# jaswon/osu-dreamer

Measured on AMD Instinct MI355X. Metric: denoiser train-steps/sec + 50-step sample latents/sec, 1/2/4/8 MI355X, higher is better.
Workload: dtype bf16

## Files before the change

include/osu_dreamer_hip.h:

```cpp
#ifndef OSU_DREAMER_HIP_H
#define OSU_DREAMER_HIP_H

#ifdef __cplusplus
extern "C" {
#endif

enum { OD_F32 = 0, OD_BF16 = 1,
       OD_F32X3 = 2,
       OD_F32X3W = 3,
       OD_F16 = 4 };
enum { OD_EPI_NONE = 0, OD_EPI_SILU = 1 };
enum { OD_ACT_NONE = 0, OD_ACT_SILU = 1 };
enum { OD_ERR_ARG = -1, OD_ERR_ALIGN = -2, OD_ERR_UNSUPPORTED = -3, OD_ERR_COMM = -4 };

int od_version(void);
const char* od_build_source_sha(void);
const char* od_error_string(int code);

int od_gemm_nt(int dtype, const void* A, int lda, const void* W, int ldw, const float* bias, void* C, int ldc,
               int M, int N, int K, int epilogue, int accumulate, void* stream);
int od_gemm_nt_qkrope(int dtype, const void* A, int lda, const void* W, int ldw, const float* bias, void* C, int ldc, int M,
                      int N, int K, const float* wq, const float* wk, const float* table, int L, int H, int hd, float eps,
                      float q_scale, void* stream);
int od_gemm_nt_qkrope_split(int dtype, const void* A, int lda, const void* W, int ldw, const float* bias, void* C, int ldc,
                            void* qk_out, int ldqk, int qk_dtype, int M, int N, int K, const float* wq, const float* wk, const float* table,
                            int L, int H, int hd, float eps, float q_scale, void* stream);
int od_gemm_tn(int dtype, const void* G, int ldg, const void* A, int lda, float* dW, int lddw, float* dbias, int M, int N,
               int K, void* stream);
int od_gemm_tn_blocks(int dtype, const void* G, int ldg, const void* A, int lda, float* dW, int lddw, float* dbias, int M, int N,
                      int K, int n_block, int n_valid, void* stream);
int od_colsum(int dtype, const void* G, int ldg, float* out, int M, int N, void* stream);
int od_pack_weight(int dtype, const float* src, int N, int K, void* dst, int Np, int Kp, int transpose,
                   const int* row_map, void* stream);

int od_linear_small(const float* x, const float* W, const float* b, float* out, float* pre, int B, int N, int K, int act,
                    void* stream);
int od_linear_small_bwd(const float* x, const float* W, const float* pre, const float* dout, float* dpre, float* dW,
                        float* db, float* dx, int accumulate_dx, int B, int N, int K, int act, void* stream);

int od_cl_to_frames(int dtype, const float* src, void* dst, int ldd, int B, int C, int L, void* stream);
int od_proj_in(int dtype, const float* xt, const float* W, const float* bias, void* x, int ldx, int B, int E, int L,
               int D, void* stream);
int od_proj_in_bwd(int dtype, const float* xt, const void* dx, int ldx, float* dW, float* db, int B, int E, int L, int D,
                   void* stream);
int od_silu(int dtype, const void* x, void* y, long n, void* stream);
int od_silu_bwd(int dtype, const void* x, const void* dy, void* dx, long n, void* stream);

int od_rmsnorm_film(int dtype, const void* x, int ldx, const float* ssg, const void* cl, int ldcl, int cl_bcast,
                    void* h, int ldh, float* inv_rms, int B, int L, int C, float eps, void* stream);
int od_rmsnorm_film_bwd(int dtype, const void* x, int ldx, const float* inv_rms, const float* ssg, const void* dh,
                        int lddh, void* dres, int lddres, float* dssg, int B, int L, int C, void* stream);
int od_rmsnorm_gate_residual(int dtype, const void* x, int ldx, const void* h, int ldh, const float* ssg, void* xo,
                             int ldxo, float* inv_rms, int B, int L, int C, float eps, void* stream);
int od_rmsnorm_gate_residual_film(int dtype, const void* x, int ldx, const void* h, int ldh, const float* ssg_a, void* xo, int ldxo,
                                  float* inv_a, const float* ssg_b, const void* cl, int ldcl, int cl_bcast, void* h2, int ldh2,
                                  float* inv_b, int B, int L, int C, float eps, void* stream);
int od_rmsnorm_gate_residual_film_dwconv(int dtype, const void* x, int ldx, const void* h, int ldh, const float* ssg_a, void* xo, int ldxo,
                                         float* inv_a, const float* ssg_b, void* h2, int ldh2, float* inv_b, const float* conv_w,
                                         const float* conv_b, void* y, int ldy, int B, int L, int C, int ksize, float eps, void* stream);
int od_rmsnorm_gate_residual_bwd(int dtype, const void* h, int ldh, const float* inv_rms, const float* ssg,
                                 const void* dy, int lddy, void* dh, int lddh, float* dssg, int B, int L, int C,
                                 void* stream);

int od_rope_table(float* table, int L, int hd, void* stream);
int od_qk_norm_rope(int dtype, const void* qkv, int ldqkv, const float* wq, const float* wk, const float* table,
                    void* qk_out, int ldo, int B, int L, int H, int hd, float eps, float q_scale, void* stream);
int od_qk_norm_rope_bwd(int dtype, const void* qkv, int ldqkv, const float* wq, const float* wk, const float* table,
                        const void* dqk, int lddqk, void* dqkv, int lddqkv, float* dwq, float* dwk, int B, int L,
                        int H, int hd, float eps, float q_scale, void* stream);
int od_flash_attn_fwd(int dtype, const void* q, int ldq, const void* k, int ldk, const void* v, int ldv, void* o, int ldo,
                      float* lse, int B, int H, int L, int hd, float scale, int q_prescaled, void* stream);
int od_flash_attn_fwd_varlen(int dtype, const void* q, int ldq, const void* k, int ldk, const void* v, int ldv, void* o, int ldo,
                             float* lse, const int* lens, int B, int H, int L, int hd, float scale, int q_prescaled, void* stream);
int od_flash_attn_bwd(int dtype, const void* q, int ldq, const void* k, int ldk, const void* v, int ldv, const void* o,
                      int ldo, const void* dout, int lddo, const float* lse, float* delta, void* dq, int lddq, void* dk,
                      int lddk, void* dv, int lddv, int B, int H, int L, int hd, float scale, int q_prescaled, void* stream);
int od_attn_aux_create(void** aux_out);
int od_attn_aux_destroy(void* aux);
int od_flash_attn_bwd_aux(int dtype, const void* q, int ldq, const void* k, int ldk, const void* v, int ldv, const void* o,
                          int ldo, const void* dout, int lddo, const float* lse, float* delta, void* dq, int lddq, void* dk,
                          int lddk, void* dv, int lddv, int B, int H, int L, int hd, float scale, int q_prescaled, void* aux, void* stream);
int od_flash_attn_bwd_fused_ws_bytes(int dtype, int B, int H, int L, long* total_out, long* zero_out);
int od_flash_attn_bwd_fused(int dtype, const void* q, int ldq, const void* k, int ldk, const void* v, int ldv, const void* o, int ldo,
                            const void* dout, int lddo, const float* lse, void* dq, int lddq, void* dk, int lddk, void* dv, int lddv,
                            int B, int H, int L, int hd, float scale, int q_prescaled, void* ws, long ws_bytes, void* stream);
int od_flash_attn_bwd_fused_status(const void* ws, int* err_out, void* stream);
int od_flash_attn_bwd_fused_err_offset(void);
int od_flash_attn_bwd_fused_passes(void);
int od_flash_attn_bwd_fused_prof(void* ws, long* out16);
int od_flash_attn_bwd_passes(void);

int od_dwconv(int dtype, const void* x, int ldx, const float* w, const float* bias, void* y, int ldy, int B, int L,
              int C, int ksize, void* stream);
int od_dwconv_varlen(int dtype, const void* x, int ldx, const float* w, const float* bias, void* y, int ldy, const int* lens,
                     int B, int L, int C, int ksize, void* stream);
int od_dwconv_bwd(int dtype, const void* x, int ldx, const float* w, const void* dy, int lddy, void* dx, int lddx,
                  float* dw, float* db, int B, int L, int C, int ksize, void* stream);
int od_scale_channels(int dtype, void* x, int ldx, const float* scale, int B, int L, int C, void* stream);
int od_swiglu_rmsnorm(int dtype, const void* vg, int ldvg, void* hh, int ldhh, float* inv_rms, int M, int Hf, int Hp,
                      float eps, void* stream);
int od_swiglu_rmsnorm_bwd(int dtype, const void* vg, int ldvg, const float* inv_rms, const void* dhh, int lddhh,
                          void* dvg, int lddvg, int M, int Hf, int Hp, void* stream);

int od_final_norm_proj_out(int dtype, const void* x, int ldx, const float* W, const float* bias, float* v,
                           float* inv_rms, int B, int L, int C, int E, float eps, void* stream);
int od_final_norm_proj_out_bwd(int dtype, const void* x, int ldx, const float* inv_rms, const float* W, const float* dv,
                               void* dx, int lddx, float* dW, float* db, int B, int L, int C, int E, void* stream);
int od_uhead_fwd(const float* xt, const float* w0, const float* b0, const float* w1, const float* b1, const float* w3,
                 const float* b3, const float* w4, const float* b4, float* fsum, int B, int E, int L, int U,
                 void* stream);
int od_uhead_fwd_varlen(const float* xt, const float* w0, const float* b0, const float* w1, const float* b1, const float* w3,
                        const float* b3, const float* w4, const float* b4, float* fsum, const int* lens, int B, int E, int L,
                        int U, void* stream);
int od_uhead_bwd(const float* xt, const float* w0, const float* b0, const float* w1, const float* b1, const float* w3,
                 const float* b3, const float* w4, const float* b4, const float* dfm, float* dw0, float* db0, float* dw1,
                 float* db1, float* dw3, float* db3, float* dw4, float* db4, int B, int E, int L, int U, void* stream);
int od_uhead_tail(const float* fsum, const float* mod, const float* w_out, const float* b_out, float* u, int B, int U,
                  int L, float u_scale, void* stream);
int od_uhead_tail_varlen(const float* fsum, const float* mod, const float* w_out, const float* b_out, float* u, const int* lens,
                         int B, int U, int L, float u_scale, void* stream);
int od_uhead_tail_bwd(const float* fsum, const float* mod, const float* w_out, const float* b_out, const float* du,
                      float* dfm, float* dmod, float* dw_out, float* db_out, int B, int U, int L, float u_scale,
                      void* stream);

int od_make_xt(const float* x0, const float* x1, const float* t, float* xt, float* dsq, int B, int E, int L, void* stream);
int od_loss_grad(const float* xt, const float* x1, const float* u, const float* v, const float* dsq, float* dv,
                 float* sums, int B, int E, int L, float c0, float osl_w, float del_w, void* stream);
int od_loss_finalize(const float* sums, const float* dsq, const float* u, float* out, float* du, int B, float c0,
                     float osl_w, float del_w, void* stream);
int od_sampler_step(float* x, const float* u, const float* v, const float* eta, int B, int E, int L, void* stream);
int od_sampler_eta(const float* u, float* eta, int B, float c0, int num_steps, void* stream);
int od_sampler_eta_groups(const float* u, const int* offs, float* eta, int G, float c0, int num_steps, void* stream);
int od_sampler_step_varlen(float* x, const float* u, const float* v, const float* eta, const int* lens, const int* offs, int G,
                           int B, int E, int L, void* stream);

int od_det_clear(void);
int od_det_register(const float* base, long count, void* shadow_i64);
int od_det_enable(void* table_dev, void* stream);
int od_det_table_bytes(void);
int od_det_flush(float* dst, long count, void* stream);

int od_sqnorm(const float* g, long n, float* out, const int* status, void* stream);
int od_adamw_ema(float* p, const float* g, float* m, float* v, float* ema, long n, float lr, float beta1, float beta2,
                 float eps, float weight_decay, int step, float ema_decay, int ema_mode, const float* gnorm_sq,
                 float max_norm, const int* status, void* stream);

int od_ema_update(float* ema, const float* p, long n, float ema_decay, int ema_mode, void* stream);

int od_style_conditioning(const float* labels, const float* rff_w, const float* rff_b, const float* cond_w,
                          const float* cond_b, const float* null_labels, float* c, int B, int NL, int F, int H,
                          void* stream);
int od_rmsnorm_rows(const float* x, const float* gamma, float* y, int M, int C, float eps, void* stream);

int od_style_conditioning_bwd(const float* labels, const float* rff_w, const float* rff_b, const float* dc, float* dcond_w,
                              float* dcond_b, float* dnull_labels, int B, int NL, int F, int H, void* stream);
int od_rmsnorm_rows_bwd(const float* x, const float* gamma, const float* dy, float* dx, float* dgamma, int M, int C, float eps,
                        int accumulate_dx, void* stream);
int od_cast_rows(int src_dtype, const void* src, int dst_dtype, void* dst, long n, void* stream);

int od_spec_features_conv(int dtype, const float* audio, const float* w1, const float* b1, const float* g1, const float* w2,
                          const float* b2, const float* g2, void* out, int ldo, int B, int F, int L, float eps, void* stream);
int od_rmsnorm_affine_film(int dtype, const void* x, int ldx, const float* gamma, const float* ssg, void* y, int ldy, int B,
                           int L, int C, float eps, int act, void* stream);
int od_rmsnorm_affine_gate_residual(int dtype, const void* x, int ldx, const void* h, int ldh, const float* gamma,
                                    const float* ssg, void* xo, int ldxo, int B, int L, int C, float eps, void* stream);
int od_unet_mixer(int dtype, const void* x, int ldx, const void* p, int ldp, int p_bcast, const void* gx, int ldg,
                  const float* gamma, void* xo, int ldxo, int B, int L, int C, float eps, void* stream);
int od_unet_down(int dtype, const void* x, int ldx, const float* w, const float* bias, void* y, int ldy, int B, int Lo, int C,
                 int stride, void* stream);
int od_unet_up(int dtype, const void* x, int ldx, const float* w, const float* bias, void* y, int ldy, int B, int Li, int C,
               int stride, void* stream);
int od_chart_head(int dtype, const void* x, int ldx, const float* W, const float* bias, float* out, int B, int L, int C, int N,
                  int n_sigmoid, int rms, float eps, void* stream);
int od_attn_pool(int dtype, const void* scores, int lds, const void* values, int ldv, float* out, int B, int L, int Hh, int hd,
                 void* stream);
int od_latent_bwd_block_frames(int C);
int od_rmsnorm_affine_film_bwd(int dtype, const void* x, int ldx, const float* gamma, const float* ssg, const void* dy, int lddy, void* dx,
                               int lddx, int accumulate_dx, float* dgamma, float* dssg, float* ws, long ws_floats, int B, int L, int C,
                               float eps, int act, void* stream);
int od_rmsnorm_affine_gate_residual_bwd(int dtype, const void* h, int ldh, const float* gamma, const float* ssg, const void* dxo, int lddxo,
                                        void* dh, int lddh, float* dgamma, float* dssg, float* ws, long ws_floats, int B, int L, int C,
                                        float eps, void* stream);
int od_unet_mixer_bwd(int dtype, const void* p, int ldp, int p_bcast, const void* gx, int ldg, const float* gamma, const void* dxo,
                      int lddxo, void* dp, int lddp, void* dgx, int lddg, float* dgamma, float* ws, long ws_floats, int B, int L, int C,
                      float eps, void* stream);
int od_unet_down_bwd(int dtype, const void* x, int ldx, const float* w, const void* dy, int lddy, void* dx, int lddx, float* dw, float* db,
                     float* ws, long ws_floats, int B, int Lo, int C, int stride, void* stream);
int od_unet_up_bwd(int dtype, const void* x, int ldx, const float* w, const void* dy, int lddy, void* dx, int lddx, float* dw, float* db,
                   float* ws, long ws_floats, int B, int Li, int C, int stride, void* stream);
int od_chart_head_bwd(int dtype, const void* x, int ldx, const float* W, const float* bias, const float* dout, void* dx, int lddx,
                      float* dW, float* db, float* ws, long ws_floats, int B, int L, int C, int N, int rms, float eps, void* stream);
int od_attn_pool_bwd(int dtype, const void* scores, int lds, const void* values, int ldv, const float* dout, void* dscores, int ldds,
                     void* dvalues, int lddv, int B, int L, int Hh, int hd, void* stream);
int od_spec_features_conv_bwd(int dtype, const float* audio, const float* w1, const float* b1, const float* g1, const float* w2,
                              const float* b2, const float* g2, const void* dout, int ldo, float* dw1, float* db1, float* dg1, float* dw2,
                              float* db2, float* dg2, float* ws, long ws_floats, int B, int F, int L, float eps, void* stream);
int od_add_rows(int dtype, const void* x, void* y, long n, void* stream);
int od_proj_in_bwd_input(int dtype, const void* dx, int ldx, const float* W, float* dxt, int B, int E, int L, int D, void* stream);

int od_mmd_imq(const float* z, const float* prior, float* out, float* dz, float* ws, long ws_floats, int N, int D, void* stream);
int od_scale_by(const float* x, const float* g, float* y, long n, void* stream);
int od_latent_perturb(const float* z, long zsb, long zse, long zsl, const float* s, const float* eps_z, const float* eps_s,
                      const float* u_s, const float* repl, const float* u_span, const float* u_start, float* z_out, float* s_out,
                      void* masked, void* start_span, int B2, int E, int l, int S, float s_noise, float z_noise, float s_mask_frac,
                      float z_mask_frac, int training, void* stream);
int od_latent_perturb_bwd(const float* dz_out, const float* ds_out, const void* masked, const int* start_span, float* dz, float* ds,
                          int B2, int E, int l, int S, void* stream);
int od_latent_loss_block_frames(void);
int od_latent_loss_ws_floats(int B2, int L);
int od_latent_loss(const float* logits, const float* chart, const float* pred_labels, const float* true_labels, const void* masked,
                   const float* s_reg, float* loss_ema, void* ema_init, float* out, float* coef, float* ws, long ws_floats, int B2, int L,
                   float s_reg_weight, int training, void* stream);
int od_latent_loss_bwd(const float* logits, const float* chart, const float* pred_labels, const float* true_labels, const void* masked,
                       const float* coef, const float* g, float* dlogits, float* dlabels, float* ds_reg, int B2, int L,
                       float s_reg_weight, void* stream);

int od_spec_features_conv_varlen(int dtype, const float* audio, const float* w1, const float* b1, const float* g1, const float* w2,
                                 const float* b2, const float* g2, void* out, int ldo, const int* lens, int B, int F, int L, float eps,
                                 void* stream);
int od_rmsnorm_affine_film_varlen(int dtype, const void* x, int ldx, const float* gamma, const float* ssg, void* y, int ldy,
                                  const int* lens, int B, int L, int C, float eps, int act, void* stream);
int od_unet_mixer_varlen(int dtype, const void* x, int ldx, const void* p, int ldp, const int* prow, const void* gx, int ldg,
                         const float* gamma, void* xo, int ldxo, int B, int L, int C, float eps, void* stream);
int od_unet_down_varlen(int dtype, const void* x, int ldx, const float* w, const float* bias, void* y, int ldy, const int* lens,
                        int B, int Lo, int C, int stride, void* stream);
int od_unet_up_varlen(int dtype, const void* x, int ldx, const float* w, const float* bias, void* y, int ldy, const int* lens,
                      int B, int Li, int C, int stride, void* stream);
int od_chart_head_varlen(int dtype, const void* x, int ldx, const float* W, const float* bias, float* out, const int* lens, int B,
                         int L, int C, int N, int n_sigmoid, int rms, float eps, void* stream);
int od_attn_pool_varlen(int dtype, const void* scores, int lds, const void* values, int ldv, float* out, const int* lens, int B,
                        int L, int Hh, int hd, void* stream);

int od_comm_load(const char* path);
int od_comm_version(void);
int od_comm_unique_id(void* out, int nbytes);
int od_comm_init(void** comm_out, int nranks, int rank, const void* unique_id, int nbytes);
int od_comm_destroy(void* comm);
int od_comm_abort(void* comm);
int od_comm_count(void* comm);
int od_comm_ring_standin(float* buf, long count, int channels, int threads, int rounds, void* stream);
int od_allreduce_grads(void* comm, float* grads, long count, int average, void* stream);
int od_broadcast_f32(void* comm, float* buf, long count, int root, void* stream);

int od_graph_begin(void* stream);
int od_graph_end(void* stream, void** graph_exec_out);
int od_graph_launch(void* graph_exec, void* stream);
int od_graph_destroy(void* graph_exec);

int od_mfma_calibrate(float* scratch, int iters, double* flops_out, void* stream);

#ifdef __cplusplus
}
#endif
#endif
```

osu_dreamer_amd/csrc/rowops.hip:

```cpp
#include "od_common.h"
#include "od_api_internal.h"

namespace {

#ifndef OD_QK_BPW
#define OD_QK_BPW 8
#endif
constexpr int ROWS_PER_WAVE_BWD = 16;

template <class T, int NCH>
__device__ __forceinline__ void load_row(const T* row, int C, int lane, float (&v)[NCH][8]) {
#pragma unroll
    for (int i = 0; i < NCH; i++) {
        const int c = (lane + 64 * i) * 8;
        if (c < C) od_ld8(row + c, v[i]);
        else {
#pragma unroll
            for (int e = 0; e < 8; e++) v[i][e] = 0.f;
        }
    }
}
template <int NCH>
__device__ __forceinline__ float row_sumsq(const float (&v)[NCH][8]) {
    float s = 0.f;
#pragma unroll
    for (int i = 0; i < NCH; i++)
#pragma unroll
        for (int e = 0; e < 8; e++) s += v[i][e] * v[i][e];
    return od_wave_sum(s);
}

template <class T, int NCH>
__global__ __launch_bounds__(256) void rmsnorm_film_kernel(const T* __restrict__ x, int ldx, const float* __restrict__ ssg,
                                                           const T* __restrict__ cl, int ldcl, int cl_bcast,
                                                           T* __restrict__ h, int ldh, float* __restrict__ inv_rms,
                                                           int B, int L, int C, float eps) {
    const int lane = threadIdx.x & 63;
    const long m = (long)blockIdx.x * 4 + (threadIdx.x >> 6);
    if (m >= (long)B * L) return;
    const int b = (int)(m / L), l = (int)(m % L);
    float v[NCH][8];
    load_row<T, NCH>(x + m * ldx, C, lane, v);
    const float inv = rsqrtf(row_sumsq<NCH>(v) / (float)C + eps);
    if (lane == 0 && inv_rms) inv_rms[m] = inv;
    const float* sc = ssg + (size_t)b * 3 * C;
    const T* clrow = cl ? cl + (size_t)(cl_bcast ? l : m) * ldcl : nullptr;
#pragma unroll
    for (int i = 0; i < NCH; i++) {
        const int c = (lane + 64 * i) * 8;
        if (c >= C) continue;
        float s[8], sh[8], o[8];
        od_ld8(sc + c, s); od_ld8(sc + C + c, sh);
#pragma unroll
        for (int e = 0; e < 8; e++) o[e] = v[i][e] * inv * (1.f + s[e]) + sh[e];
        if (clrow) {
            float a[8]; od_ld8(clrow + c, a);
#pragma unroll
            for (int e = 0; e < 8; e++) o[e] += a[e];
        }
        od_st8(h + m * ldh + c, o);
    }
}

template <class T, int NCH>
__global__ __launch_bounds__(256) void rmsnorm_film_bwd_kernel(const T* __restrict__ x, int ldx, const float* __restrict__ inv_rms,
                                                               const float* __restrict__ ssg, const T* __restrict__ dh, int lddh,
                                                               T* __restrict__ dres, int lddres, float* __restrict__ dssg,
                                                               int B, int L, int C, const OdDetTable* __restrict__ det) {
    __shared__ float red[2][NCH * 512];
    const int lane = threadIdx.x & 63, wave = threadIdx.x >> 6;
    const int b = blockIdx.y;
    const int l0 = (blockIdx.x * 4 + wave) * ROWS_PER_WAVE_BWD;
    float dsc[NCH][8], dsh[NCH][8], scl[NCH][8];
#pragma unroll
    for (int i = 0; i < NCH; i++) {
        const int c = (lane + 64 * i) * 8;
#pragma unroll
        for (int e = 0; e < 8; e++) { dsc[i][e] = 0.f; dsh[i][e] = 0.f; scl[i][e] = 0.f; }
        if (c < C) od_ld8(ssg + (size_t)b * 3 * C + c, scl[i]);
    }
    for (int r = 0; r < ROWS_PER_WAVE_BWD; r++) {
        const int l = l0 + r;
        if (l >= L) break;
        const long m = (long)b * L + l;
        float xv[NCH][8], gv[NCH][8];
        load_row<T, NCH>(x + m * ldx, C, lane, xv);
        load_row<T, NCH>(dh + m * lddh, C, lane, gv);
        const float inv = inv_rms[m];
        float dot = 0.f;
#pragma unroll
        for (int i = 0; i < NCH; i++)
#pragma unroll
            for (int e = 0; e < 8; e++) {
                const float xh = xv[i][e] * inv;
                dsc[i][e] += gv[i][e] * xh;
                dsh[i][e] += gv[i][e];
                gv[i][e] *= (1.f + scl[i][e]);
                dot += gv[i][e] * xh;
                xv[i][e] = xh;
            }
        dot = od_wave_sum(dot) / (float)C;
#pragma unroll
        for (int i = 0; i < NCH; i++) {
            const int c = (lane + 64 * i) * 8;
            if (c >= C) continue;
            float o[8];
            od_ld8(dres + m * lddres + c, o);
#pragma unroll
            for (int e = 0; e < 8; e++) o[e] += inv * (gv[i][e] - xv[i][e] * dot);
            od_st8(dres + m * lddres + c, o);
        }
    }
    for (int w = 0; w < 4; w++) {
        if (wave == w) {
#pragma unroll
            for (int i = 0; i < NCH; i++)
#pragma unroll
                for (int e = 0; e < 8; e++) {
                    const int idx = (lane + 64 * i) * 8 + e;
                    if (w == 0) { red[0][idx] = dsc[i][e]; red[1][idx] = dsh[i][e]; }
                    else { red[0][idx] += dsc[i][e]; red[1][idx] += dsh[i][e]; }
                }
        }
        __syncthreads();
    }
    for (int c = threadIdx.x; c < C; c += 256) {
        od_red_add(det, dssg + (size_t)b * 3 * C + c, red[0][c]);
        od_red_add(det, dssg + (size_t)b * 3 * C + C + c, red[1][c]);
    }
}

template <class T, int NCH>
__global__ __launch_bounds__(256) void rmsnorm_gate_res_kernel(const T* __restrict__ x, int ldx, const T* __restrict__ h, int ldh,
                                                               const float* __restrict__ ssg, T* __restrict__ xo, int ldxo,
                                                               float* __restrict__ inv_rms, int B, int L, int C, float eps) {
    const int lane = threadIdx.x & 63;
    const long m = (long)blockIdx.x * 4 + (threadIdx.x >> 6);
    if (m >= (long)B * L) return;
    const int b = (int)(m / L);
    float v[NCH][8];
    load_row<T, NCH>(h + m * ldh, C, lane, v);
    const float inv = rsqrtf(row_sumsq<NCH>(v) / (float)C + eps);
    if (lane == 0 && inv_rms) inv_rms[m] = inv;
    const float* gate = ssg + (size_t)b * 3 * C + 2 * C;
#pragma unroll
    for (int i = 0; i < NCH; i++) {
        const int c = (lane + 64 * i) * 8;
        if (c >= C) continue;
        float g[8], o[8];
        od_ld8(gate + c, g);
        od_ld8(x + m * ldx + c, o);
#pragma unroll
        for (int e = 0; e < 8; e++) o[e] += v[i][e] * inv * g[e];
        od_st8(xo + m * ldxo + c, o);
    }
}

template <class T, int NCH>
__global__ __launch_bounds__(256) void rmsnorm_gate_res_film_kernel(const T* __restrict__ x, int ldx, const T* __restrict__ h, int ldh,
                                                                    const float* __restrict__ ssg_a, T* __restrict__ xo, int ldxo,
                                                                    float* __restrict__ inv_a, const float* __restrict__ ssg_b,
                                                                    const T* __restrict__ cl, int ldcl, int cl_bcast,
                                                                    T* __restrict__ h2, int ldh2, float* __restrict__ inv_b,
                                                                    int B, int L, int C, float eps) {
    const int lane = threadIdx.x & 63;
    const long m = (long)blockIdx.x * 4 + (threadIdx.x >> 6);
    if (m >= (long)B * L) return;
    const int b = (int)(m / L), l = (int)(m % L);
    float v[NCH][8];
    load_row<T, NCH>(h + m * ldh, C, lane, v);
    const float inv = rsqrtf(row_sumsq<NCH>(v) / (float)C + eps);
    if (lane == 0 && inv_a) inv_a[m] = inv;
    const float* gate = ssg_a + (size_t)b * 3 * C + 2 * C;
#pragma unroll
    for (int i = 0; i < NCH; i++) {
        const int c = (lane + 64 * i) * 8;
        if (c >= C) {
#pragma unroll
            for (int e = 0; e < 8; e++) v[i][e] = 0.f;
            continue;
        }
        float g[8], o[8];
        od_ld8(gate + c, g);
        od_ld8(x + m * ldx + c, o);
#pragma unroll
        for (int e = 0; e < 8; e++) o[e] += v[i][e] * inv * g[e];
        od_st8(xo + m * ldxo + c, o);
#pragma unroll
        for (int e = 0; e < 8; e++) v[i][e] = od_round_to<T>(o[e]);
    }
    const float inv2 = rsqrtf(row_sumsq<NCH>(v) / (float)C + eps);
    if (lane == 0 && inv_b) inv_b[m] = inv2;
    const float* sc = ssg_b + (size_t)b * 3 * C;
    const T* clrow = cl ? cl + (size_t)(cl_bcast ? l : m) * ldcl : nullptr;
#pragma unroll
    for (int i = 0; i < NCH; i++) {
        const int c = (lane + 64 * i) * 8;
        if (c >= C) continue;
        float s2[8], sh[8], o[8];
        od_ld8(sc + c, s2); od_ld8(sc + C + c, sh);
#pragma unroll
        for (int e = 0; e < 8; e++) o[e] = v[i][e] * inv2 * (1.f + s2[e]) + sh[e];
        if (clrow) {
            float a[8]; od_ld8(clrow + c, a);
#pragma unroll
            for (int e = 0; e < 8; e++) o[e] += a[e];
        }
        od_st8(h2 + m * ldh2 + c, o);
    }
}

template <class T, int KS, int RUN>
__global__ __launch_bounds__(256) void rmsnorm_gate_res_film_dwconv_kernel(const T* __restrict__ x, int ldx, const T* __restrict__ h, int ldh,
                                                                           const float* __restrict__ ssg_a, T* __restrict__ xo, int ldxo,
                                                                           float* __restrict__ inv_a, const float* __restrict__ ssg_b,
                                                                           T* __restrict__ h2, int ldh2, float* __restrict__ inv_b,
                                                                           const float* __restrict__ cw, const float* __restrict__ cb,
                                                                           T* __restrict__ y, int ldy, int B, int L, int C, float eps) {
    constexpr int R = KS / 2;
    const int lane = threadIdx.x & 63;
    const int b = blockIdx.y;
    const int l0 = (blockIdx.x * 4 + (threadIdx.x >> 6)) * RUN;
    if (l0 >= L) return;
    const int c = lane * 8;
    const bool act = c < C;
    float gate[8], sc[8], sh[8], wv[8][KS], bv[8];
#pragma unroll
    for (int e = 0; e < 8; e++) {
        gate[e] = 0.f; sc[e] = 0.f; sh[e] = 0.f; bv[e] = 0.f;
#pragma unroll
        for (int j = 0; j < KS; j++) wv[e][j] = 0.f;
    }
    if (act) {
        od_ld8(ssg_a + (size_t)b * 3 * C + 2 * C + c, gate);
        od_ld8(ssg_b + (size_t)b * 3 * C + c, sc);
        od_ld8(ssg_b + (size_t)b * 3 * C + C + c, sh);
#pragma unroll
        for (int k = 0; k < 8; k++) {
            bv[k] = cb[c + k];
#pragma unroll
            for (int j = 0; j < KS; j++) wv[k][j] = cw[(size_t)(c + k) * KS + j];
        }
    }
    float win[KS][8];
#pragma unroll
    for (int j = 0; j < KS; j++)
#pragma unroll
        for (int e = 0; e < 8; e++) win[j][e] = 0.f;
    const int lend = l0 + RUN < L ? l0 + RUN : L;
    for (int l = l0 - R; l < lend + R; l++) {
#pragma unroll
        for (int e = 0; e < 8; e++) win[KS - 1][e] = 0.f;
        if (l >= 0 && l < L) {
            const long m = (long)b * L + l;
            const bool own = l >= l0 && l < lend;
            float v[1][8], o[8];
            load_row<T, 1>(h + m * ldh, C, lane, v);
            const float inv = rsqrtf(row_sumsq<1>(v) / (float)C + eps);
            if (act) {
                od_ld8(x + m * ldx + c, o);
#pragma unroll
                for (int e = 0; e < 8; e++) o[e] += v[0][e] * inv * gate[e];
                if (own) od_st8(xo + m * ldxo + c, o);
#pragma unroll
                for (int e = 0; e < 8; e++) v[0][e] = od_round_to<T>(o[e]);
            }
            const float inv2 = rsqrtf(row_sumsq<1>(v) / (float)C + eps);
            if (own && lane == 0) {
                if (inv_a) inv_a[m] = inv;
                if (inv_b) inv_b[m] = inv2;
            }
            if (act) {
                float hv[8];
#pragma unroll
                for (int e = 0; e < 8; e++) hv[e] = v[0][e] * inv2 * (1.f + sc[e]) + sh[e];
                if (own && h2) od_st8(h2 + m * ldh2 + c, hv);
#pragma unroll
                for (int e = 0; e < 8; e++) win[KS - 1][e] = od_round_to<T>(hv[e]);
            }
        }
        const int lc = l - R;
        if (lc >= l0 && lc < lend && act) {
            float o[8];
#pragma unroll
            for (int k = 0; k < 8; k++) {
                float s = bv[k];
#pragma unroll
                for (int j = 0; j < KS; j++) s += wv[k][j] * win[j][k];
                o[k] = s;
            }
            od_st8(y + ((size_t)b * L + lc) * ldy + c, o);
        }
#pragma unroll
        for (int j = 0; j < KS - 1; j++)
#pragma unroll
            for (int e = 0; e < 8; e++) win[j][e] = win[j + 1][e];
    }
}

template <class T, int NCH>
__global__ __launch_bounds__(256) void rmsnorm_gate_res_bwd_kernel(const T* __restrict__ h, int ldh, const float* __restrict__ inv_rms,
                                                                   const float* __restrict__ ssg, const T* __restrict__ dy, int lddy,
                                                                   T* __restrict__ dh, int lddh, float* __restrict__ dssg,
                                                                   int B, int L, int C, const OdDetTable* __restrict__ det) {
    __shared__ float red[NCH * 512];
    const int lane = threadIdx.x & 63, wave = threadIdx.x >> 6;
    const int b = blockIdx.y;
    const int l0 = (blockIdx.x * 4 + wave) * ROWS_PER_WAVE_BWD;
    float dg[NCH][8], gate[NCH][8];
#pragma unroll
    for (int i = 0; i < NCH; i++) {
        const int c = (lane + 64 * i) * 8;
#pragma unroll
        for (int e = 0; e < 8; e++) { dg[i][e] = 0.f; gate[i][e] = 0.f; }
        if (c < C) od_ld8(ssg + (size_t)b * 3 * C + 2 * C + c, gate[i]);
    }
    for (int r = 0; r < ROWS_PER_WAVE_BWD; r++) {
        const int l = l0 + r;
        if (l >= L) break;
        const long m = (long)b * L + l;
        float hv[NCH][8], gv[NCH][8];
        load_row<T, NCH>(h + m * ldh, C, lane, hv);
        load_row<T, NCH>(dy + m * lddy, C, lane, gv);
        const float inv = inv_rms[m];
        float dot = 0.f;
#pragma unroll
        for (int i = 0; i < NCH; i++)
#pragma unroll
            for (int e = 0; e < 8; e++) {
                const float hh = hv[i][e] * inv;
                dg[i][e] += gv[i][e] * hh;
                gv[i][e] *= gate[i][e];
                dot += gv[i][e] * hh;
                hv[i][e] = hh;
            }
        dot = od_wave_sum(dot) / (float)C;
#pragma unroll
        for (int i = 0; i < NCH; i++) {
            const int c = (lane + 64 * i) * 8;
            if (c >= C) continue;
            float o[8];
#pragma unroll
            for (int e = 0; e < 8; e++) o[e] = inv * (gv[i][e] - hv[i][e] * dot);
            od_st8(dh + m * lddh + c, o);
        }
    }
    for (int w = 0; w < 4; w++) {
        if (wave == w) {
#pragma unroll
            for (int i = 0; i < NCH; i++)
#pragma unroll
                for (int e = 0; e < 8; e++) {
                    const int idx = (lane + 64 * i) * 8 + e;
                    if (w == 0) red[idx] = dg[i][e]; else red[idx] += dg[i][e];
                }
        }
        __syncthreads();
    }
    for (int c = threadIdx.x; c < C; c += 256) od_red_add(det, dssg + (size_t)b * 3 * C + 2 * C + c, red[c]);
}

template <class T, int NCH>
__global__ __launch_bounds__(256) void swiglu_rmsnorm_kernel(const T* __restrict__ vg, int ldvg, T* __restrict__ hh, int ldhh,
                                                             float* __restrict__ inv_rms, long M, int Hf, int Hp, float eps) {
    const int lane = threadIdx.x & 63;
    const long m = (long)blockIdx.x * 4 + (threadIdx.x >> 6);
    if (m >= M) return;
    float v[NCH][8], g[NCH][8];
    load_row<T, NCH>(vg + m * ldvg, Hp, lane, v);
    load_row<T, NCH>(vg + m * ldvg + Hp, Hp, lane, g);
#pragma unroll
    for (int i = 0; i < NCH; i++)
#pragma unroll
        for (int e = 0; e < 8; e++) v[i][e] *= od_silu(g[i][e]);
    const float inv = rsqrtf(row_sumsq<NCH>(v) / (float)Hf + eps);
    if (lane == 0 && inv_rms) inv_rms[m] = inv;
#pragma unroll
    for (int i = 0; i < NCH; i++) {
        const int c = (lane + 64 * i) * 8;
        if (c >= Hp) continue;
        float o[8];
#pragma unroll
        for (int e = 0; e < 8; e++) o[e] = v[i][e] * inv;
        od_st8(hh + m * ldhh + c, o);
    }
}

template <class T, int NCH>
__global__ __launch_bounds__(256) void swiglu_rmsnorm_bwd_kernel(const T* __restrict__ vg, int ldvg, const float* __restrict__ inv_rms,
                                                                 const T* __restrict__ dhh, int lddhh, T* __restrict__ dvg, int lddvg,
                                                                 long M, int Hf, int Hp) {
    const int lane = threadIdx.x & 63;
    const long m = (long)blockIdx.x * 4 + (threadIdx.x >> 6);
    if (m >= M) return;
    float v[NCH][8], g[NCH][8], d[NCH][8];
    load_row<T, NCH>(vg + m * ldvg, Hp, lane, v);
    load_row<T, NCH>(vg + m * ldvg + Hp, Hp, lane, g);
    load_row<T, NCH>(dhh + m * lddhh, Hp, lane, d);
    const float inv = inv_rms[m];
    float dot = 0.f;
    float sg[NCH][8], gs[NCH][8];
#pragma unroll
    for (int i = 0; i < NCH; i++)
#pragma unroll
        for (int e = 0; e < 8; e++) {
            gs[i][e] = od_sigmoid(g[i][e]);
            sg[i][e] = g[i][e] * gs[i][e];
            dot += d[i][e] * (v[i][e] * sg[i][e] * inv);
        }
    dot = od_wave_sum(dot) / (float)Hf;
#pragma unroll
    for (int i = 0; i < NCH; i++) {
        const int c = (lane + 64 * i) * 8;
        if (c >= Hp) continue;
        float ov[8], og[8];
#pragma unroll
        for (int e = 0; e < 8; e++) {
            const float sh = v[i][e] * sg[i][e] * inv;
            const float ds = inv * (d[i][e] - sh * dot);
            ov[e] = ds * sg[i][e];
            og[e] = ds * v[i][e] * (gs[i][e] * (1.0f + g[i][e] * (1.0f - gs[i][e])));
        }
        od_st8(dvg + m * lddvg + c, ov);
        od_st8(dvg + m * lddvg + Hp + c, og);
    }
}

template <class T, int NCH>
__global__ __launch_bounds__(256) void final_proj_kernel(const T* __restrict__ x, int ldx, const float* __restrict__ W,
                                                         const float* __restrict__ bias, float* __restrict__ vout,
                                                         float* __restrict__ inv_rms, int B, int L, int C, int E, float eps) {
    const int lane = threadIdx.x & 63;
    const long m = (long)blockIdx.x * 4 + (threadIdx.x >> 6);
    if (m >= (long)B * L) return;
    const int b = (int)(m / L), l = (int)(m % L);
    float v[NCH][8];
    load_row<T, NCH>(x + m * ldx, C, lane, v);
    const float inv = rsqrtf(row_sumsq<NCH>(v) / (float)C + eps);
    if (lane == 0 && inv_rms) inv_rms[m] = inv;
    for (int e = 0; e < E; e++) {
        float s = 0.f;
#pragma unroll
        for (int i = 0; i < NCH; i++) {
            const int c = (lane + 64 * i) * 8;
            if (c >= C) continue;
            float w[8]; od_ld8(W + (size_t)e * C + c, w);
#pragma unroll
            for (int k = 0; k < 8; k++) s += w[k] * v[i][k];
        }
        s = od_wave_sum(s) * inv;
        if (lane == 0) vout[((size_t)b * E + e) * L + l] = s + bias[e];
    }
}

template <class T, int NCH>
__global__ __launch_bounds__(256) void final_proj_bwd_kernel(const T* __restrict__ x, int ldx, const float* __restrict__ inv_rms,
                                                             const float* __restrict__ W, const float* __restrict__ dv,
                                                             T* __restrict__ dx, int lddx, float* __restrict__ dW,
                                                             float* __restrict__ db, int B, int L, int C, int E,
                                                             const OdDetTable* __restrict__ det) {
    constexpr int MAXE = 8;
    __shared__ float red[MAXE * NCH * 512];
    __shared__ float redb[4][MAXE];
    const int lane = threadIdx.x & 63, wave = threadIdx.x >> 6;
    const int b = blockIdx.y;
    const int l0 = (blockIdx.x * 4 + wave) * ROWS_PER_WAVE_BWD;
    float wv[MAXE][NCH][8], dw[MAXE][NCH][8], dbv[MAXE];
#pragma unroll
    for (int e = 0; e < MAXE; e++) {
        dbv[e] = 0.f;
#pragma unroll
        for (int i = 0; i < NCH; i++) {
            const int c = (lane + 64 * i) * 8;
#pragma unroll
            for (int k = 0; k < 8; k++) { wv[e][i][k] = 0.f; dw[e][i][k] = 0.f; }
            if (e < E && c < C) od_ld8(W + (size_t)e * C + c, wv[e][i]);
        }
    }
    for (int r = 0; r < ROWS_PER_WAVE_BWD; r++) {
        const int l = l0 + r;
        if (l >= L) break;
        const long m = (long)b * L + l;
        float xv[NCH][8], dn[NCH][8], dve[MAXE];
        load_row<T, NCH>(x + m * ldx, C, lane, xv);
        const float inv = inv_rms[m];
#pragma unroll
        for (int e = 0; e < MAXE; e++) { dve[e] = e < E ? dv[((size_t)b * E + e) * L + l] : 0.f; dbv[e] += dve[e]; }
        float dot = 0.f;
#pragma unroll
        for (int i = 0; i < NCH; i++)
#pragma unroll
            for (int k = 0; k < 8; k++) {
                const float xh = xv[i][k] * inv;
                float s = 0.f;
#pragma unroll
                for (int e = 0; e < MAXE; e++) { s += dve[e] * wv[e][i][k]; dw[e][i][k] += dve[e] * xh; }
                dn[i][k] = s;
                dot += s * xh;
                xv[i][k] = xh;
            }
        dot = od_wave_sum(dot) / (float)C;
#pragma unroll
        for (int i = 0; i < NCH; i++) {
            const int c = (lane + 64 * i) * 8;
            if (c >= C) continue;
            float o[8];
#pragma unroll
            for (int k = 0; k < 8; k++) o[k] = inv * (dn[i][k] - xv[i][k] * dot);
            od_st8(dx + m * lddx + c, o);
        }
    }
    if (lane == 0)
        for (int e = 0; e < MAXE; e++) redb[wave][e] = dbv[e];
    for (int w = 0; w < 4; w++) {
        if (wave == w) {
#pragma unroll
            for (int e = 0; e < MAXE; e++)
#pragma unroll
                for (int i = 0; i < NCH; i++)
#pragma unroll
                    for (int k = 0; k < 8; k++) {
                        const int idx = e * NCH * 512 + (lane + 64 * i) * 8 + k;
                        if (w == 0) red[idx] = dw[e][i][k]; else red[idx] += dw[e][i][k];
                    }
        }
        __syncthreads();
    }
    for (int e = 0; e < E; e++)
        for (int c = threadIdx.x; c < C; c += 256) od_red_add(det, dW + (size_t)e * C + c, red[e * NCH * 512 + c]);
    if (threadIdx.x < E) od_red_add(det, db + threadIdx.x, redb[0][threadIdx.x] + redb[1][threadIdx.x] + redb[2][threadIdx.x] + redb[3][threadIdx.x]);
}

template <class T, class TO = T>
__global__ __launch_bounds__(256) void qk_norm_rope_kernel(const T* __restrict__ qkv, int ldqkv, const float* __restrict__ wq,
                                                           const float* __restrict__ wk, const float* __restrict__ table,
                                                           TO* __restrict__ out, int ldo, int B, int L, int H, int hd, float eps,
                                                           float q_scale) {
    const int lane = threadIdx.x & 63;
    const long m = (long)blockIdx.x * 4 + (threadIdx.x >> 6);
    if (m >= (long)B * L) return;
    const int l = (int)(m % L);
    const int lph = hd / 8, half = lph / 2;
    const int nchunks = 2 * H * lph;
    const int niter = (nchunks + 63) / 64;
    for (int it = 0; it < niter; it++) {
        const int q = it * 64 + lane;
        const bool act = q < nchunks;
        const int slot = q / lph, c8 = q % lph;
        float v[8];
        if (act) od_ld8(qkv + m * ldqkv + (size_t)slot * hd + c8 * 8, v);
        else {
#pragma unroll
            for (int e = 0; e < 8; e++) v[e] = 0.f;
        }
        float ss = 0.f;
#pragma unroll
        for (int e = 0; e < 8; e++) ss += v[e] * v[e];
        for (int msk = 1; msk < lph; msk <<= 1) ss += __shfl_xor(ss, msk);
        const float inv = rsqrtf(ss / (float)hd + eps);
        const float* w = (slot < H ? wq : wk) + c8 * 8;
        float y[8], p[8];
#pragma unroll
        for (int e = 0; e < 8; e++) y[e] = act ? v[e] * inv * w[e] : 0.f;
#pragma unroll
        for (int e = 0; e < 8; e++) p[e] = __shfl_xor(y[e], half);
        if (act) {
            const bool first = c8 < half;
            const int j0 = (c8 % half) * 8;
            const float* tb = table + ((size_t)l * (hd / 2) + j0) * 2;
            float o[8];
#pragma unroll
            for (int e = 0; e < 8; e++) {
                const float cs = tb[2 * e], sn = tb[2 * e + 1];
                o[e] = (first ? (y[e] * cs - p[e] * sn) : (p[e] * sn + y[e] * cs)) * (slot < H ? q_scale : 1.f);
            }
            od_st8(out + m * ldo + (size_t)slot * hd + c8 * 8, o);
        }
    }
}

template <class T>
__global__ __launch_bounds__(256) void qk_norm_rope_bwd_kernel(const T* __restrict__ qkv, int ldqkv, const float* __restrict__ wq,
                                                               const float* __restrict__ wk, const float* __restrict__ table,
                                                               const T* __restrict__ dqk, int lddqk, T* __restrict__ dqkv, int lddqkv,
                                                               float* __restrict__ dwq, float* __restrict__ dwk,
                                                               int B, int L, int H, int hd, float eps, float q_scale,
                                                               const OdDetTable* __restrict__ det) {
    __shared__ long long sdw[2][256];
    __shared__ int s_bad;
    const int lane = threadIdx.x & 63, wave = threadIdx.x >> 6;
    for (int i = threadIdx.x; i < 512; i += 256) sdw[i >> 8][i & 255] = 0;
    if (threadIdx.x == 0) s_bad = 0;
    __syncthreads();
    const int lph = hd / 8, half = lph / 2;
    const int nchunks = 2 * H * lph;
    const int niter = (nchunks + 63) / 64;
    float aq[8], ak[8];
#pragma unroll
    for (int e = 0; e < 8; e++) { aq[e] = 0.f; ak[e] = 0.f; }
    const long M = (long)B * L;
    const long mbase = ((long)blockIdx.x * 4 + wave) * ROWS_PER_WAVE_BWD;
    for (int r = 0; r < ROWS_PER_WAVE_BWD; r++) {
        const long m = mbase + r;
        if (m >= M) break;
        const int l = (int)(m % L);
        for (int it = 0; it < niter; it++) {
            const int q = it * 64 + lane;
            const bool act = q < nchunks;
            const int slot = q / lph, c8 = q % lph;
            float v[8], d[8];
            if (act) {
                od_ld8(qkv + m * ldqkv + (size_t)slot * hd + c8 * 8, v); od_ld8(dqk + m * lddqk + (size_t)slot * hd + c8 * 8, d);
                if (slot < H) {
#pragma unroll
                    for (int e = 0; e < 8; e++) d[e] *= q_scale;
                }
            } else {
#pragma unroll
                for (int e = 0; e < 8; e++) { v[e] = 0.f; d[e] = 0.f; }
            }
            float ss = 0.f;
#pragma unroll
            for (int e = 0; e < 8; e++) ss += v[e] * v[e];
            for (int msk = 1; msk < lph; msk <<= 1) ss += __shfl_xor(ss, msk);
            const float inv = rsqrtf(ss / (float)hd + eps);
            float p[8], dy[8];
#pragma unroll
            for (int e = 0; e < 8; e++) p[e] = __shfl_xor(d[e], half);
            const bool first = c8 < half;
            const int j0 = (c8 % (half > 0 ? half : 1)) * 8;
            const float* tb = table + ((size_t)l * (hd / 2) + j0) * 2;
            const float* w = (slot < H ? wq : wk) + c8 * 8;
            float dot = 0.f;
#pragma unroll
            for (int e = 0; e < 8; e++) {
                const float cs = act ? tb[2 * e] : 0.f, sn = act ? tb[2 * e + 1] : 0.f;
                dy[e] = first ? (d[e] * cs + p[e] * sn) : (-p[e] * sn + d[e] * cs);
                const float xh = v[e] * inv;
                const float wv = act ? w[e] : 0.f;
                if (act) { if (slot < H) aq[e] += dy[e] * xh; else ak[e] += dy[e] * xh; }
                dy[e] *= wv;
                dot += dy[e] * xh;
                v[e] = xh;
            }
            for (int msk = 1; msk < lph; msk <<= 1) dot += __shfl_xor(dot, msk);
            dot /= (float)hd;
            if (act) {
                float o[8];
#pragma unroll
                for (int e = 0; e < 8; e++) o[e] = inv * (dy[e] - v[e] * dot);
                od_st8(dqkv + m * lddqkv + (size_t)slot * hd + c8 * 8, o);
            }
        }
    }
    const int c8 = lane % lph;
#pragma unroll
    for (int e = 0; e < 8; e++) {
        od_lds_fix_add(&sdw[0][c8 * 8 + e], aq[e], &s_bad);
        od_lds_fix_add(&sdw[1][c8 * 8 + e], ak[e], &s_bad);
    }
    __syncthreads();
    if (threadIdx.x < hd) {
        od_red_add(det, dwq + threadIdx.x, od_lds_unfix(sdw[0][threadIdx.x], s_bad));
        od_red_add(det, dwk + threadIdx.x, od_lds_unfix(sdw[1][threadIdx.x], s_bad));
    }
}

template <class T, int LPH, int NIT>
__global__ __launch_bounds__(256) void qk_norm_rope_pos_kernel(const T* __restrict__ qkv, int ldqkv, const float* __restrict__ wq,
                                                               const float* __restrict__ wk, const float* __restrict__ table,
                                                               T* __restrict__ out, int ldo, int B, int L, float eps, float q_scale,
                                                               int bpw, int lpw) {
    constexpr int HD = 8 * LPH, HALFL = LPH / 2;
    const int lane = threadIdx.x & 63, c8 = lane % LPH;
    const int wpl = (B + bpw - 1) / bpw;
    const long gw = (long)blockIdx.x * 4 + (threadIdx.x >> 6);
    const int l0 = (int)(gw / wpl) * lpw, b0 = (int)(gw % wpl) * bpw;
    if (l0 >= L) return;
    const int l1 = l0 + lpw < L ? l0 + lpw : L, b1 = b0 + bpw < B ? b0 + bpw : B;
    float w[2][8];
    od_ld8(wq + c8 * 8, w[0]); od_ld8(wk + c8 * 8, w[1]);
#pragma unroll
    for (int e = 0; e < 8; e++) w[0][e] *= q_scale;
    const bool first = c8 < HALFL;
    for (int l = l0; l < l1; l++) {
        float tb[16];
        const float* tp = table + ((size_t)l * (HD / 2) + (c8 % HALFL) * 8) * 2;
        od_ld8(tp, *(float(*)[8])&tb[0]); od_ld8(tp + 8, *(float(*)[8])&tb[8]);
        float cs[8], sn[8];
#pragma unroll
        for (int e = 0; e < 8; e++) { cs[e] = tb[2 * e]; sn[e] = first ? -tb[2 * e + 1] : tb[2 * e + 1]; }
        for (int b = b0; b < b1; b++) {
            const long m = (long)b * L + l;
            float v[NIT][8];
#pragma unroll
            for (int it = 0; it < NIT; it++) od_ld8(qkv + m * ldqkv + (size_t)(it * 64 + lane) * 8, v[it]);
#pragma unroll
            for (int it = 0; it < NIT; it++) {
                float ss = 0.f;
#pragma unroll
                for (int e = 0; e < 8; e++) ss += v[it][e] * v[it][e];
#pragma unroll
                for (int msk = 1; msk < LPH; msk <<= 1) ss += __shfl_xor(ss, msk);
                const float inv = rsqrtf(ss / (float)HD + eps);
                const float* wv = w[it < NIT / 2 ? 0 : 1];
                float y[8], o[8];
#pragma unroll
                for (int e = 0; e < 8; e++) y[e] = v[it][e] * inv * wv[e];
#pragma unroll
                for (int e = 0; e < 8; e++) o[e] = y[e] * cs[e] + __shfl_xor(y[e], HALFL) * sn[e];
                od_st8(out + m * ldo + (size_t)(it * 64 + lane) * 8, o);
            }
        }
    }
}

template <class T, int LPH, int NIT>
__global__ __launch_bounds__(256) void qk_norm_rope_pos_bwd_kernel(const T* __restrict__ qkv, int ldqkv, const float* __restrict__ wq,
                                                                   const float* __restrict__ wk, const float* __restrict__ table,
                                                                   const T* __restrict__ dqk, int lddqk, T* __restrict__ dqkv, int lddqkv,
                                                                   float* __restrict__ dwq, float* __restrict__ dwk,
                                                                   int B, int L, float eps, float q_scale, int bpw, int lpw,
                                                                   const OdDetTable* __restrict__ det) {
    constexpr int HD = 8 * LPH, HALFL = LPH / 2;
    __shared__ long long s_dw[2][HD];
    __shared__ int s_bad;
    for (int i = threadIdx.x; i < 2 * HD; i += 256) s_dw[i / HD][i % HD] = 0;
    if (threadIdx.x == 0) s_bad = 0;
    __syncthreads();
    const int lane = threadIdx.x & 63, c8 = lane % LPH;
    const int wpl = (B + bpw - 1) / bpw;
    const long gw = (long)blockIdx.x * 4 + (threadIdx.x >> 6);
    const int l0 = (int)(gw / wpl) * lpw, b0 = (int)(gw % wpl) * bpw;
    const int l1 = l0 + lpw < L ? l0 + lpw : L, b1 = b0 + bpw < B ? b0 + bpw : B;
    float w[2][8], acc[2][8];
    od_ld8(wq + c8 * 8, w[0]); od_ld8(wk + c8 * 8, w[1]);
#pragma unroll
    for (int e = 0; e < 8; e++) { acc[0][e] = 0.f; acc[1][e] = 0.f; }
    const bool first = c8 < HALFL;
    for (int l = l0; l < l1; l++) {
        float tb[16];
        const float* tp = table + ((size_t)l * (HD / 2) + (c8 % HALFL) * 8) * 2;
        od_ld8(tp, *(float(*)[8])&tb[0]); od_ld8(tp + 8, *(float(*)[8])&tb[8]);
        float cs[8], sn[8];
#pragma unroll
        for (int e = 0; e < 8; e++) { cs[e] = tb[2 * e]; sn[e] = first ? tb[2 * e + 1] : -tb[2 * e + 1]; }
        for (int b = b0; b < b1; b++) {
            const long m = (long)b * L + l;
            float v[NIT][8], d[NIT][8];
#pragma unroll
            for (int it = 0; it < NIT; it++) {
                od_ld8(qkv + m * ldqkv + (size_t)(it * 64 + lane) * 8, v[it]);
                od_ld8(dqk + m * lddqk + (size_t)(it * 64 + lane) * 8, d[it]);
            }
#pragma unroll
            for (int it = 0; it < NIT; it++) {
                const int qk = it < NIT / 2 ? 0 : 1;
                const float gs = qk == 0 ? q_scale : 1.f;
                float ss = 0.f;
#pragma unroll
                for (int e = 0; e < 8; e++) ss += v[it][e] * v[it][e];
#pragma unroll
                for (int msk = 1; msk < LPH; msk <<= 1) ss += __shfl_xor(ss, msk);
                const float inv = rsqrtf(ss / (float)HD + eps);
                float dy[8], xh[8], dot = 0.f;
#pragma unroll
                for (int e = 0; e < 8; e++) d[it][e] *= gs;
#pragma unroll
                for (int e = 0; e < 8; e++) {
                    const float u = d[it][e] * cs[e] + __shfl_xor(d[it][e], HALFL) * sn[e];
                    xh[e] = v[it][e] * inv;
                    acc[qk][e] += u * xh[e];
                    dy[e] = u * w[qk][e];
                    dot += dy[e] * xh[e];
                }
#pragma unroll
                for (int msk = 1; msk < LPH; msk <<= 1) dot += __shfl_xor(dot, msk);
                dot /= (float)HD;
                float o[8];
#pragma unroll
                for (int e = 0; e < 8; e++) o[e] = inv * (dy[e] - xh[e] * dot);
                od_st8(dqkv + m * lddqkv + (size_t)(it * 64 + lane) * 8, o);
            }
        }
    }
#pragma unroll
    for (int msk = LPH; msk < 64; msk <<= 1)
#pragma unroll
        for (int e = 0; e < 8; e++) { acc[0][e] += __shfl_xor(acc[0][e], msk); acc[1][e] += __shfl_xor(acc[1][e], msk); }
    if (lane < LPH) {
#pragma unroll
        for (int e = 0; e < 8; e++) { od_lds_fix_add(&s_dw[0][c8 * 8 + e], acc[0][e], &s_bad); od_lds_fix_add(&s_dw[1][c8 * 8 + e], acc[1][e], &s_bad); }
    }
    __syncthreads();
    if (threadIdx.x < HD) {
        od_red_add(det, dwq + threadIdx.x, od_lds_unfix(s_dw[0][threadIdx.x], s_bad));
        od_red_add(det, dwk + threadIdx.x, od_lds_unfix(s_dw[1][threadIdx.x], s_bad));
    }
}

__global__ void rope_table_kernel(float* __restrict__ table, int L, int hd) {
    const long i = (long)blockIdx.x * blockDim.x + threadIdx.x;
    const int half = hd / 2;
    if (i >= (long)L * half) return;
    const int l = (int)(i / half), j = (int)(i % half);
    const float e = (float)(2 * j) / (float)(-hd);
    const float inv_freq = (float)pow(10000.0, (double)e);
    const float ang = (float)l * inv_freq;
    table[2 * i] = cosf(ang);
    table[2 * i + 1] = sinf(ang);
}

inline int nch_for(int C) { return (C + 511) / 512; }

inline void qk_pos_split(int B, int L, int& bpw, int& lpw) {
    bpw = B < OD_QK_BPW ? B : OD_QK_BPW;
    lpw = OD_QK_BPW / bpw;
    if (lpw < 1) lpw = 1;
    (void)L;
}

}

#define DISPATCH_T_NCH(DT, NCHV, CALL)                                          \
    do {                                                                        \
        if ((DT) == OD_BF16) {                                                  \
            typedef bf16_t T_;                                                  \
            if ((NCHV) == 1) { constexpr int N_ = 1; CALL; }                    \
            else if ((NCHV) == 2) { constexpr int N_ = 2; CALL; }               \
            else if ((NCHV) == 3) { constexpr int N_ = 3; CALL; }               \
            else return OD_ERR_UNSUPPORTED;                                     \
        } else if ((DT) == OD_F32) {                                            \
            typedef float T_;                                                   \
            if ((NCHV) == 1) { constexpr int N_ = 1; CALL; }                    \
            else if ((NCHV) == 2) { constexpr int N_ = 2; CALL; }               \
            else if ((NCHV) == 3) { constexpr int N_ = 3; CALL; }               \
            else return OD_ERR_UNSUPPORTED;                                     \
        } else return OD_ERR_ARG;                                               \
    } while (0)

extern "C" int od_rmsnorm_film(int dtype, const void* x, int ldx, const float* ssg, const void* cl, int ldcl, int cl_bcast,
                               void* h, int ldh, float* inv_rms, int B, int L, int C, float eps, void* stream) {
    if (C % 8 || ldx % 8 || ldh % 8 || (cl && ldcl % 8)) return OD_ERR_ALIGN;
    const long M = (long)B * L;
    dim3 grid((unsigned)((M + 3) / 4));
    DISPATCH_T_NCH(dtype, nch_for(C),
        OD_LAUNCH((rmsnorm_film_kernel<T_, N_>), grid, dim3(256), 0, (hipStream_t)stream, (const T_*)x, ldx, ssg, (const T_*)cl, ldcl,
                  cl_bcast, (T_*)h, ldh, inv_rms, B, L, C, eps));
    OD_CHECK_LAUNCH();
    return 0;
}

extern "C" int od_rmsnorm_film_bwd(int dtype, const void* x, int ldx, const float* inv_rms, const float* ssg, const void* dh,
                                   int lddh, void* dres, int lddres, float* dssg, int B, int L, int C, void* stream) {
    if (C % 8 || ldx % 8 || lddh % 8 || lddres % 8) return OD_ERR_ALIGN;
    dim3 grid((L + 4 * ROWS_PER_WAVE_BWD - 1) / (4 * ROWS_PER_WAVE_BWD), B);
    DISPATCH_T_NCH(dtype, nch_for(C),
        OD_LAUNCH((rmsnorm_film_bwd_kernel<T_, N_>), grid, dim3(256), 0, (hipStream_t)stream, (const T_*)x, ldx, inv_rms, ssg,
                  (const T_*)dh, lddh, (T_*)dres, lddres, dssg, B, L, C, od_det_active()));
    OD_CHECK_LAUNCH();
    return 0;
}

extern "C" int od_rmsnorm_gate_residual(int dtype, const void* x, int ldx, const void* h, int ldh, const float* ssg, void* xo,
                                        int ldxo, float* inv_rms, int B, int L, int C, float eps, void* stream) {
    if (C % 8 || ldx % 8 || ldh % 8 || ldxo % 8) return OD_ERR_ALIGN;
    const long M = (long)B * L;
    dim3 grid((unsigned)((M + 3) / 4));
    DISPATCH_T_NCH(dtype, nch_for(C),
        OD_LAUNCH((rmsnorm_gate_res_kernel<T_, N_>), grid, dim3(256), 0, (hipStream_t)stream, (const T_*)x, ldx, (const T_*)h, ldh, ssg,
                  (T_*)xo, ldxo, inv_rms, B, L, C, eps));
    OD_CHECK_LAUNCH();
    return 0;
}

extern "C" int od_rmsnorm_gate_residual_film(int dtype, const void* x, int ldx, const void* h, int ldh, const float* ssg_a, void* xo,
                                             int ldxo, float* inv_a, const float* ssg_b, const void* cl, int ldcl, int cl_bcast,
                                             void* h2, int ldh2, float* inv_b, int B, int L, int C, float eps, void* stream) {
    if (C % 8 || ldx % 8 || ldh % 8 || ldxo % 8 || ldh2 % 8 || (cl && ldcl % 8)) return OD_ERR_ALIGN;
    const long M = (long)B * L;
    dim3 grid((unsigned)((M + 3) / 4));
    DISPATCH_T_NCH(dtype, nch_for(C),
        OD_LAUNCH((rmsnorm_gate_res_film_kernel<T_, N_>), grid, dim3(256), 0, (hipStream_t)stream, (const T_*)x, ldx, (const T_*)h, ldh,
                  ssg_a, (T_*)xo, ldxo, inv_a, ssg_b, (const T_*)cl, ldcl, cl_bcast, (T_*)h2, ldh2, inv_b, B, L, C, eps));
    OD_CHECK_LAUNCH();
    return 0;
}

extern "C" int od_rmsnorm_gate_residual_film_dwconv(int dtype, const void* x, int ldx, const void* h, int ldh, const float* ssg_a, void* xo,
                                                    int ldxo, float* inv_a, const float* ssg_b, void* h2, int ldh2, float* inv_b,
                                                    const float* conv_w, const float* conv_b, void* y, int ldy, int B, int L, int C,
                                                    int ksize, float eps, void* stream) {
    if (C % 8 || ldx % 8 || ldh % 8 || ldxo % 8 || (h2 && ldh2 % 8) || ldy % 8) return OD_ERR_ALIGN;
    if (C > 512 || (ksize != 3 && ksize != 5 && ksize != 7 && ksize != 9)) return OD_ERR_UNSUPPORTED;
    if (!x || !h || !xo || !y || !conv_w || !conv_b || xo == x || xo == h) return OD_ERR_ARG;
#ifndef OD_FD_SMALL_RUNS
#define OD_FD_SMALL_RUNS 2048
#endif
    const bool small = (long)B * ((L + 31) / 32) < OD_FD_SMALL_RUNS;
    const int run = small ? 8 : 32;
    dim3 grid((unsigned)((L + 4 * run - 1) / (4 * run)), (unsigned)B);
#define FD_GO2(T_, KS_, RUN_) OD_LAUNCH((rmsnorm_gate_res_film_dwconv_kernel<T_, KS_, RUN_>), grid, dim3(256), 0, (hipStream_t)stream, (const T_*)x, ldx, \
                   (const T_*)h, ldh, ssg_a, (T_*)xo, ldxo, inv_a, ssg_b, (T_*)h2, ldh2, inv_b, conv_w, conv_b, (T_*)y, ldy, B, L, C, eps)
#define FD_GO1(T_, KS_) do { if (small) FD_GO2(T_, KS_, 8); else FD_GO2(T_, KS_, 32); } while (0)
#define FD_GO(KS_) do { if (dtype == OD_BF16) FD_GO1(bf16_t, KS_); else if (dtype == OD_F32) FD_GO1(float, KS_); else return OD_ERR_UNSUPPORTED; } while (0)
    if (ksize == 5) FD_GO(5); else if (ksize == 3) FD_GO(3); else if (ksize == 7) FD_GO(7); else FD_GO(9);
#undef FD_GO
#undef FD_GO1
#undef FD_GO2
    OD_CHECK_LAUNCH();
    return 0;
}

extern "C" int od_rmsnorm_gate_residual_bwd(int dtype, const void* h, int ldh, const float* inv_rms, const float* ssg,
                                            const void* dy, int lddy, void* dh, int lddh, float* dssg, int B, int L, int C,
                                            void* stream) {
    if (C % 8 || ldh % 8 || lddy % 8 || lddh % 8) return OD_ERR_ALIGN;
    dim3 grid((L + 4 * ROWS_PER_WAVE_BWD - 1) / (4 * ROWS_PER_WAVE_BWD), B);
    DISPATCH_T_NCH(dtype, nch_for(C),
        OD_LAUNCH((rmsnorm_gate_res_bwd_kernel<T_, N_>), grid, dim3(256), 0, (hipStream_t)stream, (const T_*)h, ldh, inv_rms, ssg,
                  (const T_*)dy, lddy, (T_*)dh, lddh, dssg, B, L, C, od_det_active()));
    OD_CHECK_LAUNCH();
    return 0;
}

extern "C" int od_swiglu_rmsnorm(int dtype, const void* vg, int ldvg, void* hh, int ldhh, float* inv_rms, int M, int Hf, int Hp,
                                 float eps, void* stream) {
    if (Hp % 8 || ldvg % 8 || ldhh % 8 || Hf > Hp) return OD_ERR_ALIGN;
    dim3 grid((unsigned)((M + 3) / 4));
    DISPATCH_T_NCH(dtype, nch_for(Hp),
        OD_LAUNCH((swiglu_rmsnorm_kernel<T_, N_>), grid, dim3(256), 0, (hipStream_t)stream, (const T_*)vg, ldvg, (T_*)hh, ldhh, inv_rms,
                  (long)M, Hf, Hp, eps));
    OD_CHECK_LAUNCH();
    return 0;
}

extern "C" int od_swiglu_rmsnorm_bwd(int dtype, const void* vg, int ldvg, const float* inv_rms, const void* dhh, int lddhh,
                                     void* dvg, int lddvg, int M, int Hf, int Hp, void* stream) {
    if (Hp % 8 || ldvg % 8 || lddhh % 8 || lddvg % 8 || Hf > Hp) return OD_ERR_ALIGN;
    dim3 grid((unsigned)((M + 3) / 4));
    DISPATCH_T_NCH(dtype, nch_for(Hp),
        OD_LAUNCH((swiglu_rmsnorm_bwd_kernel<T_, N_>), grid, dim3(256), 0, (hipStream_t)stream, (const T_*)vg, ldvg, inv_rms,
                  (const T_*)dhh, lddhh, (T_*)dvg, lddvg, (long)M, Hf, Hp));
    OD_CHECK_LAUNCH();
    return 0;
}

extern "C" int od_final_norm_proj_out(int dtype, const void* x, int ldx, const float* W, const float* bias, float* v,
                                      float* inv_rms, int B, int L, int C, int E, float eps, void* stream) {
    if (C % 8 || ldx % 8) return OD_ERR_ALIGN;
    if (E > 8 || C > 1024) return OD_ERR_UNSUPPORTED;
    const long M = (long)B * L;
    dim3 grid((unsigned)((M + 3) / 4));
    DISPATCH_T_NCH(dtype, nch_for(C),
        OD_LAUNCH((final_proj_kernel<T_, N_>), grid, dim3(256), 0, (hipStream_t)stream, (const T_*)x, ldx, W, bias, v, inv_rms, B, L, C, E, eps));
    OD_CHECK_LAUNCH();
    return 0;
}

extern "C" int od_final_norm_proj_out_bwd(int dtype, const void* x, int ldx, const float* inv_rms, const float* W,
                                          const float* dv, void* dx, int lddx, float* dW, float* db, int B, int L, int C, int E,
                                          void* stream) {
    if (C % 8 || ldx % 8 || lddx % 8) return OD_ERR_ALIGN;
    if (E > 8 || C > 512) return OD_ERR_UNSUPPORTED;
    dim3 grid((L + 4 * ROWS_PER_WAVE_BWD - 1) / (4 * ROWS_PER_WAVE_BWD), B);
    if (dtype == OD_BF16)
        OD_LAUNCH((final_proj_bwd_kernel<bf16_t, 1>), grid, dim3(256), 0, (hipStream_t)stream, (const bf16_t*)x, ldx, inv_rms, W, dv,
                  (bf16_t*)dx, lddx, dW, db, B, L, C, E, od_det_active());
    else
        OD_LAUNCH((final_proj_bwd_kernel<float, 1>), grid, dim3(256), 0, (hipStream_t)stream, (const float*)x, ldx, inv_rms, W, dv,
                  (float*)dx, lddx, dW, db, B, L, C, E, od_det_active());
    OD_CHECK_LAUNCH();
    return 0;
}

extern "C" int od_rope_table(float* table, int L, int hd, void* stream) {
    if (hd % 2 || L <= 0) return OD_ERR_ARG;
    const long n = (long)L * (hd / 2);
    OD_LAUNCH(rope_table_kernel, dim3((unsigned)((n + 255) / 256)), dim3(256), 0, (hipStream_t)stream, table, L, hd);
    OD_CHECK_LAUNCH();
    return 0;
}

extern "C" int od_qk_norm_rope(int dtype, const void* qkv, int ldqkv, const float* wq, const float* wk, const float* table,
                               void* qk_out, int ldo, int B, int L, int H, int hd, float eps, float q_scale, void* stream) {
    if (hd % 16 || hd > 256 || 64 % (hd / 8)) return OD_ERR_UNSUPPORTED;
    if (ldqkv % 8 || ldo % 8) return OD_ERR_ALIGN;
    const long M = (long)B * L;
    const int lph = hd / 8;
    if (dtype != OD_F16 && (lph == 4 || lph == 8) && (H * lph) % 64 == 0 && ldqkv >= 2 * H * hd) {
        const int nit = 2 * H * lph / 64;
        if (nit == 2 || nit == 4 || nit == 8) {
            int bpw, lpw; qk_pos_split(B, L, bpw, lpw);
            const long waves = (long)((L + lpw - 1) / lpw) * ((B + bpw - 1) / bpw);
            dim3 g2((unsigned)((waves + 3) / 4));
#define QKP(TT, LPHV, NITV) OD_LAUNCH((qk_norm_rope_pos_kernel<TT, LPHV, NITV>), g2, dim3(256), 0, (hipStream_t)stream, (const TT*)qkv, ldqkv, wq, wk, table, (TT*)qk_out, ldo, B, L, eps, q_scale, bpw, lpw)
#define QKP_T(TT) do { if (lph == 8) { if (nit == 2) QKP(TT, 8, 2); else if (nit == 4) QKP(TT, 8, 4); else QKP(TT, 8, 8); } \
                       else { if (nit == 2) QKP(TT, 4, 2); else if (nit == 4) QKP(TT, 4, 4); else QKP(TT, 4, 8); } } while (0)
            if (dtype == OD_BF16) QKP_T(bf16_t); else QKP_T(float);
#undef QKP_T
#undef QKP
            OD_CHECK_LAUNCH();
            return 0;
        }
    }
    dim3 grid((unsigned)((M + 3) / 4));
    if (dtype == OD_F16)
        OD_LAUNCH((qk_norm_rope_kernel<bf16_t, f16_t>), grid, dim3(256), 0, (hipStream_t)stream, (const bf16_t*)qkv, ldqkv, wq, wk, table,
                  (f16_t*)qk_out, ldo, B, L, H, hd, eps, q_scale);
    else if (dtype == OD_BF16)
        OD_LAUNCH((qk_norm_rope_kernel<bf16_t>), grid, dim3(256), 0, (hipStream_t)stream, (const bf16_t*)qkv, ldqkv, wq, wk, table,
                  (bf16_t*)qk_out, ldo, B, L, H, hd, eps, q_scale);
    else
        OD_LAUNCH((qk_norm_rope_kernel<float>), grid, dim3(256), 0, (hipStream_t)stream, (const float*)qkv, ldqkv, wq, wk, table,
                  (float*)qk_out, ldo, B, L, H, hd, eps, q_scale);
    OD_CHECK_LAUNCH();
    return 0;
}

extern "C" int od_qk_norm_rope_bwd(int dtype, const void* qkv, int ldqkv, const float* wq, const float* wk, const float* table,
                                   const void* dqk, int lddqk, void* dqkv, int lddqkv, float* dwq, float* dwk, int B, int L,
                                   int H, int hd, float eps, float q_scale, void* stream) {
    if (hd % 16 || hd > 256 || 64 % (hd / 8)) return OD_ERR_UNSUPPORTED;
    if (ldqkv % 8 || lddqk % 8 || lddqkv % 8) return OD_ERR_ALIGN;
    const long M = (long)B * L;
    const int lph = hd / 8;
    if ((lph == 4 || lph == 8) && (H * lph) % 64 == 0) {
        const int nit = 2 * H * lph / 64;
        if (nit == 2 || nit == 4 || nit == 8) {
            int bpw, lpw; qk_pos_split(B, L, bpw, lpw);
            lpw *= 4;
            const long waves = (long)((L + lpw - 1) / lpw) * ((B + bpw - 1) / bpw);
            dim3 g2((unsigned)((waves + 3) / 4));
#define QKPB(TT, LPHV, NITV) OD_LAUNCH((qk_norm_rope_pos_bwd_kernel<TT, LPHV, NITV>), g2, dim3(256), 0, (hipStream_t)stream, (const TT*)qkv, ldqkv, wq, wk, table, (const TT*)dqk, lddqk, (TT*)dqkv, lddqkv, dwq, dwk, B, L, eps, q_scale, bpw, lpw, od_det_active())
#define QKPB_T(TT) do { if (lph == 8) { if (nit == 2) QKPB(TT, 8, 2); else if (nit == 4) QKPB(TT, 8, 4); else QKPB(TT, 8, 8); } \
                        else { if (nit == 2) QKPB(TT, 4, 2); else if (nit == 4) QKPB(TT, 4, 4); else QKPB(TT, 4, 8); } } while (0)
            if (dtype == OD_BF16) QKPB_T(bf16_t); else QKPB_T(float);
#undef QKPB_T
#undef QKPB
            OD_CHECK_LAUNCH();
            return 0;
        }
    }
    dim3 grid((unsigned)((M + 4 * ROWS_PER_WAVE_BWD - 1) / (4 * ROWS_PER_WAVE_BWD)));
    if (dtype == OD_BF16)
        OD_LAUNCH((qk_norm_rope_bwd_kernel<bf16_t>), grid, dim3(256), 0, (hipStream_t)stream, (const bf16_t*)qkv, ldqkv, wq, wk, table,
                  (const bf16_t*)dqk, lddqk, (bf16_t*)dqkv, lddqkv, dwq, dwk, B, L, H, hd, eps, q_scale, od_det_active());
    else
        OD_LAUNCH((qk_norm_rope_bwd_kernel<float>), grid, dim3(256), 0, (hipStream_t)stream, (const float*)qkv, ldqkv, wq, wk, table,
                  (const float*)dqk, lddqk, (float*)dqkv, lddqkv, dwq, dwk, B, L, H, hd, eps, q_scale, od_det_active());
    OD_CHECK_LAUNCH();
    return 0;
}
```

osu_dreamer_amd/engine.py:

```python
from __future__ import annotations


import math
import os
from typing import Dict, List, Optional

import torch

from . import det, ops
from ._lib import OD_ACT_NONE, OD_ACT_SILU

OD_FUSE_FILM_DWCONV_DEFAULT = "0"

FP32_EPS = float(torch.finfo(torch.float32).eps)


def _ceil(x: int, m: int) -> int:
    return (x + m - 1) // m * m


class Workspace:

    def __init__(self, device):
        self.device = device
        self.t: Dict[str, torch.Tensor] = {}
        self.bytes = 0

    def get(self, name: str, shape, dtype) -> torch.Tensor:
        t = self.t.get(name)
        if t is None:
            t = torch.zeros(shape, dtype=dtype, device=self.device)
            self.t[name] = t
            self.bytes += t.numel() * t.element_size()
            if name in det.WS_NAMES:
                ctx = det.context(self.device)
                if ctx is not None:
                    ctx.register(t)
        return t


class DenoiserEngine:
    def __init__(self, model):
        self.model = model
        a = model.args
        ba = a.backbone_args
        self.E, self.A, self.S = model.emb_dim, model.a_dim, model.style_dim
        self.Cg, self.D, self.U = a.global_cond_dim, a.backbone_dim, a.u_head_dim
        self.H, self.hd, self.depth = ba.n_heads, ba.head_dim, ba.depth
        self.dh = self.H * self.hd
        self.q_scale = math.log2(math.e) / math.sqrt(self.hd)
        self.radius = ba.radius
        self.ksize = 1 + 2 * ba.radius
        self.Hf = int(self.D * ba.expand * 2 / 3)
        self.Hp = _ceil(self.Hf, 64)
        if ba.radius not in (0, 1, 2, 3, 4):
            raise NotImplementedError("depthwise kernel sizes 3, 5, 7, 9 (radius 1-4) are compiled; radius 0 is the identity")
        if not (0.0 <= ba.dropout < 1.0):
            raise ValueError(f"dropout probability has to be in [0, 1), got {ba.dropout}")
        self.dropout = float(ba.dropout)
        self._packed: Dict[str, torch.Tensor] = {}
        self._packed_key = None
        self._plan_key = None
        self.ws: Optional[Workspace] = None
        self._rowmap = None
        self.generation = 0
        self._attn_aux = None
        self._attn_ws_cache: Dict[tuple, "ops.FusedAttnBwdWorkspace"] = {}
        self._attn_ws = None
        self.varlen = False
        self.attn_f16 = False

    def _det_flush(self, *tensors):
        ctx = det.context(self.model.arena.data.device)
        if ctx is not None:
            for t in tensors:
                ctx.flush(t)

    def _det_flush_segment(self, name: str):
        ctx = det.context(self.model.arena.data.device)
        if ctx is not None:
            s, e = self.model.arena.segments(self.depth)[name]
            ctx.flush(self.model.arena.ensure_grad()[s:e])

    def P(self, name: str) -> torch.Tensor:
        return self.model.arena.view(name)

    def G(self, name: str) -> torch.Tensor:
        return self.model.arena.grad_view(name)

    def _gemm_weights(self) -> List[str]:
        names = ["proj_audio.0"]
        for i in range(self.depth):
            p = f"net.layers.{i}."
            names += [p + "proj_cl", p + "attn.qkv_proj", p + "attn.out_proj", p + "ffn.proj_vg.1", p + "ffn.proj_o"]
        return names

    def pack_weights(self, dtype: torch.dtype, train: bool, x3: bool = False):
        dev = self.model.arena.data.device
        x3 = bool(x3 and dtype == torch.float32 and not train)
        key = (dtype, train, dev, x3)
        if self._packed_key != key:
            self._packed = {}
            self._packed_key = key
            self.generation += 1
            Hf, Hp = self.Hf, self.Hp
            rm = [-1] * (2 * Hp)
            for j in range(Hf):
                rm[j] = j
                rm[Hp + j] = Hf + j
            self._rowmap = torch.tensor(rm, dtype=torch.int32, device=dev)
        pk = self._packed
        for n in self._gemm_weights():
            w = self.P(n + ".weight")
            N, K = w.shape[0], w.shape[1]
            Np, Kp, rmap = N, K, None
            if n.endswith("ffn.proj_vg.1"):
                Np, rmap = 2 * self.Hp, self._rowmap
            if n.endswith("ffn.proj_o"):
                Kp = self.Hp
            if n not in pk:
                pk[n] = torch.empty(Np, Kp, dtype=dtype, device=dev)
                if x3 and Kp % 32 == 0:
                    pk[n] = ops.SplitWeight(pk[n])
                if train:
                    pk[n + ".T"] = torch.empty(Kp, Np, dtype=dtype, device=dev)
                if rmap is not None:
                    pk[n + ".b"] = torch.empty(Np, dtype=torch.float32, device=dev)
            ops.pack_weight(w, pk[n], row_map=rmap)
            if train:
                ops.pack_weight(w, pk[n + ".T"], transpose=True, row_map=rmap)
            if rmap is not None:
                ops.pack_weight(self.P(n + ".bias"), pk[n + ".b"].view(Np, 1), row_map=rmap)

    def W(self, name: str, T: bool = False) -> torch.Tensor:
        return self._packed[name + (".T" if T else "")]

    def plain_gemm(self, A: torch.Tensor, W: torch.Tensor, bias, C: torch.Tensor):
        ops.gemm_nt(A, W, bias, C, x3=self.x3)

    def plan(self, B: int, L: int, Ba: int, dtype: torch.dtype, train: bool, x3: bool = False, lens=None, offs=None):
        dev = self.model.arena.data.device
        assert not (x3 and train), "the f32x3 product exists for the forward kernels only"
        varlen = lens is not None
        assert not (varlen and train), "the varlen forward exists for no-grad paths only"
        x3 = bool(x3 and dtype == torch.float32)
        ngroups = len(offs) - 1 if offs is not None else 0
        key = (B, L, Ba, dtype, train, dev, x3, getattr(self.model, "attn_dtype", None), varlen, ngroups)
        if key != self._plan_key:
            self.ws = Workspace(dev)
            self._plan_key = key
            self.generation += 1
            tab = self.ws.get("rope", (L, self.hd // 2, 2), torch.float32)
            ops.rope_table(tab, L, self.hd)
        self.varlen = varlen
        if varlen:
            lens_t = torch.as_tensor(lens).to("cpu", torch.int32)
            if lens_t.shape != (B,) or int(lens_t.min()) < 1 or int(lens_t.max()) > L:
                raise ValueError(f"lens must hold B = {B} lengths in [1, {L}]")
            self.ws.get("vl.lens", (B,), torch.int32).copy_(lens_t)
            if offs is not None:
                offs_t = torch.as_tensor(offs).to("cpu", torch.int32)
                if int(offs_t[0]) != 0 or int(offs_t[-1]) != B or bool((offs_t[1:] <= offs_t[:-1]).any()):
                    raise ValueError("offs must rise strictly from 0 to B")
                self.ws.get("vl.offs", (ngroups + 1,), torch.int32).copy_(offs_t)
        self.B, self.L, self.Ba, self.dtype, self.train, self.x3 = B, L, Ba, dtype, train, x3
        self.M, self.Ma = B * L, Ba * L
        self.attn_f16 = getattr(self.model, "attn_dtype", None) == torch.float16
        if self.attn_f16 and (dtype != torch.bfloat16 or self.hd != 64):
            if not getattr(self, "_warned_f16_fallback", False):
                import warnings
                warnings.warn(f"attn_dtype = float16 applies to compute_dtype bfloat16 with head_dim 64; this plan (dtype {dtype}, head_dim "
                              f"{self.hd}) runs its attention in {dtype}")
                self._warned_f16_fallback = True
            self.attn_f16 = False
        return self.ws

    def buf(self, name, shape, dtype=None):
        return self.ws.get(name, shape, self.dtype if dtype is None else dtype)

    def lbuf(self, name, i, shape, dtype=None):
        return self.buf(f"{name}.{i}" if self.train else name, shape, dtype)

    def conditioning(self, audio: torch.Tensor, style: torch.Tensor):
        B, Ba, L = self.B, self.Ba, self.L
        D, A, Cg, U = self.D, self.A, self.Cg, self.U
        f32 = torch.float32
        a_t = self.buf("a_t", (self.Ma, A))
        a_pre = self.buf("a_pre", (self.Ma, A))
        a = self.buf("a", (self.Ma, A))
        ops.cl_to_frames(audio, a_t)
        ops.gemm_nt(a_t, self.W("proj_audio.0"), self.P("proj_audio.0.bias"), a_pre, x3=self.x3)
        ops.silu(a_pre, a)
        cg, cg_pre = self.buf("cg", (B, Cg), f32), self.buf("cg_pre", (B, Cg), f32)
        ops.linear_small(style, self.P("proj_style.0.weight"), self.P("proj_style.0.bias"), cg, cg_pre, OD_ACT_SILU)
        for i in range(self.depth):
            p = f"net.layers.{i}."
            for s in ("ssg1", "ssg2"):
                ops.linear_small(cg, self.P(p + s + ".weight"), self.P(p + s + ".bias"),
                                 self.buf(f"{s}.{i}", (B, 3 * D), f32))
            if not self.train:
                ops.gemm_nt(a, self.W(p + "proj_cl"), self.P(p + "proj_cl.bias"), self.buf(f"cl.{i}", (self.Ma, D)), x3=self.x3)
        ops.linear_small(cg, self.P("u_mod.weight"), self.P("u_mod.bias"), self.buf("umod", (B, 2 * U), f32))

    def pred(self, xt: torch.Tensor, u: torch.Tensor, v: torch.Tensor):
        B, L, M, D, dh, Hp = self.B, self.L, self.M, self.D, self.dh, self.Hp
        f32 = torch.float32
        tab = self.ws.t["rope"]
        bcast = self.Ba == 1 and B > 1
        x = self.lbuf("x_in", 0, (M, D))
        ops.proj_in(xt, self.P("proj_in.weight"), self.P("proj_in.bias"), x)

        def cl_of(i):
            if not self.train:
                return self.ws.t[f"cl.{i}"]
            cl = self.buf("cl", (self.Ma, D))
            ops.gemm_nt(self.ws.t["a"], self.W(f"net.layers.{i}.proj_cl"), self.P(f"net.layers.{i}.proj_cl.bias"), cl)
            return cl

        h1 = self.lbuf("h1", 0, (M, D))
        ops.rmsnorm_film(x, self.ws.t["ssg1.0"], cl_of(0), bcast, h1, self.lbuf("inv1", 0, (M,), f32), B, L)
        for i in range(self.depth):
            p = f"net.layers.{i}."
            ssg1, ssg2 = self.ws.t[f"ssg1.{i}"], self.ws.t[f"ssg2.{i}"]
            qkv = self.lbuf("qkv", i, (M, 3 * dh))
            if self.train or self.attn_f16 or self.hd not in (32, 64) or (2 * dh) % 128:
                qk = self.lbuf("qk16" if self.attn_f16 else "qk", i, (M, 2 * dh), torch.float16 if self.attn_f16 else None)
                ops.gemm_nt_qkrope_split(h1, self.W(p + "attn.qkv_proj"), self.P(p + "attn.qkv_proj.bias"), qkv, qk,
                                         self.P(p + "attn.q_norm.weight"), self.P(p + "attn.k_norm.weight"), tab, L, self.H,
                                         self.hd, FP32_EPS, x3=self.x3, q_scale=self.q_scale)
            else:
                ops.gemm_nt_qkrope(h1, self.W(p + "attn.qkv_proj"), self.P(p + "attn.qkv_proj.bias"), qkv,
                                   self.P(p + "attn.q_norm.weight"), self.P(p + "attn.k_norm.weight"), tab, L,
                                   self.H, self.hd, FP32_EPS, x3=self.x3, q_scale=self.q_scale)
                qk = qkv
            y = self.lbuf("y", i, (M, dh))
            lse = self.lbuf("lse", i, (B, self.H, L), f32)
            if self.varlen:
                ops.flash_attn_fwd_varlen(qk[:, :dh], qk[:, dh:], self._v_of(qkv), y, lse, self.ws.t["vl.lens"], B, self.H, L, self.hd,
                                          1.0 / math.sqrt(self.hd), x3=self.x3, q_prescaled=True)
            else:
                ops.flash_attn_fwd(qk[:, :dh], qk[:, dh:], self._v_of(qkv), y, lse, B, self.H, L, self.hd,
                                   1.0 / math.sqrt(self.hd), x3=self.x3, q_prescaled=True)
            ao = self.lbuf("ao", i, (M, D))
            self.plain_gemm(y, self.W(p + "attn.out_proj"), self.P(p + "attn.out_proj.bias"), ao)
            x_mid = self.lbuf("x_mid", i, (M, D))
            h2 = self.lbuf("h2", i, (M, D))
            fuse_dw = (self.radius > 0 and not self.varlen and D <= 512 and x.data_ptr() != x_mid.data_ptr() and x.dtype in (torch.bfloat16, torch.float32)
                       and os.environ.get("OD_FUSE_FILM_DWCONV", OD_FUSE_FILM_DWCONV_DEFAULT) == "1")
            if fuse_dw:
                hdw = self.lbuf("hdw", i, (M, D))
                ops.rmsnorm_gate_residual_film_dwconv(x, ao, ssg1, x_mid, self.lbuf("inv2", i, (M,), f32), ssg2, h2 if self.train else None,
                                                      self.lbuf("inv3", i, (M,), f32),
                                                      self.P(p + "ffn.proj_vg.0.weight"), self.P(p + "ffn.proj_vg.0.bias"), hdw, B, L, self.ksize)
            else:
                ops.rmsnorm_gate_residual_film(x, ao, ssg1, x_mid, self.lbuf("inv2", i, (M,), f32), ssg2, None, False, h2,
                                               self.lbuf("inv3", i, (M,), f32), B, L)
            if fuse_dw:
                pass
            elif self.radius > 0:
                hdw = self.lbuf("hdw", i, (M, D))
                if self.varlen:
                    ops.dwconv_varlen(h2, self.P(p + "ffn.proj_vg.0.weight"), self.P(p + "ffn.proj_vg.0.bias"), hdw, self.ws.t["vl.lens"], B, L,
                                      self.ksize)
                else:
                    ops.dwconv(h2, self.P(p + "ffn.proj_vg.0.weight"), self.P(p + "ffn.proj_vg.0.bias"), hdw, B, L, self.ksize)
            else:
                hdw = h2
            vg = self.lbuf("vg", i, (M, 2 * Hp))
            ops.gemm_nt(hdw, self.W(p + "ffn.proj_vg.1"), self._packed[p + "ffn.proj_vg.1.b"], vg, x3=self.x3)
            hh = self.lbuf("hh", i, (M, Hp))
            ops.swiglu_rmsnorm(vg, hh, self.lbuf("inv4", i, (M,), f32), self.Hf, Hp)
            if self._drop_active():
                ops.scale_channels(hh, self.draw_dropout_mask(i), B, L)
            fo = self.lbuf("fo", i, (M, D))
            self.plain_gemm(hh, self.W(p + "ffn.proj_o"), self.P(p + "ffn.proj_o.bias"), fo)
            x = self.buf(f"x_in.{i + 1}", (M, D)) if self.train else self.buf(f"x_in.{(i + 1) & 1}", (M, D))
            if i + 1 < self.depth:
                h1 = self.lbuf("h1", i + 1, (M, D))
                ops.rmsnorm_gate_residual_film(x_mid, fo, ssg2, x, self.lbuf("inv5", i, (M,), f32),
                                               self.ws.t[f"ssg1.{i + 1}"], cl_of(i + 1), bcast, h1,
                                               self.lbuf("inv1", i + 1, (M,), f32), B, L)
            else:
                ops.rmsnorm_gate_residual(x_mid, fo, ssg2, x, self.lbuf("inv5", i, (M,), f32), B, L)
        self._x_last = x
        ops.final_norm_proj_out(x, self.P("proj_out.weight"), self.P("proj_out.bias"), v,
                                self.buf("invf", (M,), f32), B, L)
        fsum = self.buf("fsum", (B, self.U), f32)
        fsum.zero_()
        if self.varlen:
            ops.uhead_fwd_varlen(xt, self._uhead_w(), fsum, self.ws.t["vl.lens"], self.U)
            self._det_flush(fsum)
            ops.uhead_tail_varlen(fsum, self.ws.t["umod"], self.P("u_out.weight"), self.P("u_out.bias"), u, self.ws.t["vl.lens"], L,
                                  self.model.u_scale)
        else:
            ops.uhead_fwd(xt, self._uhead_w(), fsum, self.U)
            self._det_flush(fsum)
            ops.uhead_tail(fsum, self.ws.t["umod"], self.P("u_out.weight"), self.P("u_out.bias"), u, L, self.model.u_scale)

    def _v_of(self, qkv: torch.Tensor) -> torch.Tensor:
        v = qkv[:, 2 * self.dh:]
        return v.view(torch.float16) if self.attn_f16 else v

    def attn_bwd_passes(self) -> int:
        from . import _lib
        return int(_lib.lib().cdll.od_flash_attn_bwd_fused_passes() if self.fused_attn_bwd() else _lib.lib().cdll.od_flash_attn_bwd_passes())

    def fused_attn_bwd(self) -> bool:
        import os
        if self.dtype != torch.bfloat16 or self.hd != 64:
            return False
        if self.attn_f16:
            return True
        env = os.environ.get("OD_ATTN_BWD_FUSED", "")
        if env in ("0", "1"):
            return env == "1"
        return self.L >= 2048

    def attn_bwd_launch(self, i: int, dy: torch.Tensor, delta: torch.Tensor, dqkv: torch.Tensor, core_only: bool = False):
        t, dh, p = self.ws.t, self.dh, f"net.layers.{i}."
        qk, qkv, y, lse = t[f"qk16.{i}" if self.attn_f16 else f"qk.{i}"], t[f"qkv.{i}"], t[f"y.{i}"], t[f"lse.{i}"]
        wq, wk = self.P(p + "attn.q_norm.weight"), self.P(p + "attn.k_norm.weight")
        gq, gk = self.G(p + "attn.q_norm.weight"), self.G(p + "attn.k_norm.weight")
        scale = 1.0 / math.sqrt(self.hd)
        dqk = self.buf("d.qk", (self.M, 2 * dh))
        if self.fused_attn_bwd():
            key = (self.B, self.H, self.L, qk.device, qk.dtype)
            ws = self._attn_ws_cache.get(key)
            if ws is None:
                if len(self._attn_ws_cache) >= 4:
                    self._attn_ws_cache.pop(next(iter(self._attn_ws_cache)))
                ws = self._attn_ws_cache[key] = ops.FusedAttnBwdWorkspace(self.B, self.H, self.L, qk.device, qk.dtype)
                ws.checked = False
            self._attn_ws = ws
            ops.flash_attn_bwd_fused(qk[:, :dh], qk[:, dh:], self._v_of(qkv), y, dy, lse, dqk[:, :dh], dqk[:, dh:], dqkv[:, 2 * dh:],
                                     self.B, self.H, self.L, self.hd, scale, self._attn_ws, q_prescaled=True)
        else:
            if (self._attn_aux is None or self._attn_aux.device != qk.device) and qk.is_cuda:
                if self._attn_aux is not None:
                    self._attn_aux.close()
                with torch.cuda.device(qk.device):
                    self._attn_aux = ops.AttnAux()
                self._attn_aux.device = qk.device
            ops.flash_attn_bwd(qk[:, :dh], qk[:, dh:], qkv[:, 2 * dh:], y, dy, lse, delta, dqk[:, :dh], dqk[:, dh:],
                               dqkv[:, 2 * dh:], self.B, self.H, self.L, self.hd, scale, q_prescaled=True, aux=self._attn_aux)
        if not core_only:
            ops.qk_norm_rope_bwd(qkv, wq, wk, t["rope"], dqk, dqkv, gq, gk, self.B, self.L, self.H, self.hd, FP32_EPS, q_scale=self.q_scale)

    def _drop_active(self) -> bool:
        return self.dropout > 0.0 and self.model.training

    def _drop_mask(self, i: int) -> torch.Tensor:
        return self.ws.t[f"drop.{i}"]

    def draw_dropout_mask(self, i: int) -> torch.Tensor:
        keep = 1.0 - self.dropout
        m = self.buf(f"drop.{i}", (self.B, self.Hp), torch.float32)
        m.zero_()
        m[:, :self.Hf] = torch.empty(self.B, self.Hf, device=m.device, dtype=torch.float32).bernoulli_(keep) / keep
        return m

    def _uhead_w(self, grads=False):
        f = self.G if grads else self.P
        return [f(f"u_head.{j}.{s}") for j in (0, 1, 3, 4) for s in ("weight", "bias")]

    def backward(self, xt: torch.Tensor, style: torch.Tensor, du: torch.Tensor, dv: torch.Tensor, reducer=None):
        assert self.train
        B, L, M, D, dh, Hf, Hp, A = self.B, self.L, self.M, self.D, self.dh, self.Hf, self.Hp, self.A
        f32 = torch.float32
        dctx = det.context(self.model.arena.data.device)
        if dctx is not None:
            dctx.register(self.model.arena.ensure_grad())
        tab = self.ws.t["rope"]
        cg, a = self.ws.t["cg"], self.ws.t["a"]
        dx = self.buf("d.x", (M, D))
        dbr = self.buf("d.branch", (M, D))
        dtmp = self.buf("d.tmp", (M, D))
        dhh = self.buf("d.hh", (M, Hp))
        dvg = self.buf("d.vg", (M, 2 * Hp))
        dy = self.buf("d.y", (M, dh))
        dqkv = self.buf("d.qkv", (M, 3 * dh))
        da = self.buf("d.a", (self.Ma, A))
        delta = self.buf("d.delta", (B, self.H, L), f32)
        dcg = self.buf("d.cg", (B, self.Cg), f32)
        dssg1, dssg2 = self.buf("d.ssg1", (B, 3 * D), f32), self.buf("d.ssg2", (B, 3 * D), f32)

        ops.final_norm_proj_out_bwd(self._x_last, self.ws.t["invf"], self.P("proj_out.weight"), dv, dx,
                                    self.G("proj_out.weight"), self.G("proj_out.bias"), B, L)
        dfm, dmod = self.buf("d.fm", (B, self.U), f32), self.buf("d.mod", (B, 2 * self.U), f32)
        ops.uhead_tail_bwd(self.ws.t["fsum"], self.ws.t["umod"], self.P("u_out.weight"), self.P("u_out.bias"), du,
                           dfm, dmod, self.G("u_out.weight"), self.G("u_out.bias"), L, self.model.u_scale)
        ops.uhead_bwd(xt, self._uhead_w(), dfm, self._uhead_w(grads=True), self.U)
        ops.linear_small_bwd(cg, self.P("u_mod.weight"), None, dmod, self.buf("d.lin_pre_umod", (B, 2 * self.U), f32),
                             self.G("u_mod.weight"), self.G("u_mod.bias"), dcg, False, OD_ACT_NONE)
        self._det_flush_segment("tail")
        if reducer is not None:
            reducer.segment_done("tail")

        for i in reversed(range(self.depth)):
            p = f"net.layers.{i}."
            t = self.ws.t
            ssg1, ssg2 = t[f"ssg1.{i}"], t[f"ssg2.{i}"]
            dssg1.zero_()
            dssg2.zero_()
            ops.rmsnorm_gate_residual_bwd(t[f"fo.{i}"], t[f"inv5.{i}"], ssg2, dx, dbr, dssg2, B, L)
            ops.gemm_tn(dbr, t[f"hh.{i}"], self.G(p + "ffn.proj_o.weight"), n_cols=D, k_cols=Hf,
                        dbias=self.G(p + "ffn.proj_o.bias"))
            ops.gemm_nt(dbr, self.W(p + "ffn.proj_o", T=True), None, dhh)
            if self._drop_active():
                ops.scale_channels(dhh, self._drop_mask(i), B, L)
            ops.swiglu_rmsnorm_bwd(t[f"vg.{i}"], t[f"inv4.{i}"], dhh, dvg, Hf, Hp)
            gw, gb = self.G(p + "ffn.proj_vg.1.weight"), self.G(p + "ffn.proj_vg.1.bias")
            hdw = t[f"hdw.{i}"] if self.radius > 0 else t[f"h2.{i}"]
            ops.gemm_tn(dvg, hdw, gw, n_cols=2 * Hp, k_cols=D, dbias=gb, n_block=Hp, n_valid=Hf)
            if self.radius > 0:
                self.plain_gemm(dvg, self.W(p + "ffn.proj_vg.1", T=True), None, dtmp)
                ops.dwconv_bwd(t[f"h2.{i}"], self.P(p + "ffn.proj_vg.0.weight"), dtmp, dbr,
                               self.G(p + "ffn.proj_vg.0.weight"), self.G(p + "ffn.proj_vg.0.bias"), B, L, self.ksize)
            else:
                self.plain_gemm(dvg, self.W(p + "ffn.proj_vg.1", T=True), None, dbr)
            ops.rmsnorm_film_bwd(t[f"x_mid.{i}"], t[f"inv3.{i}"], ssg2, dbr, dx, dssg2, B, L)
            ops.rmsnorm_gate_residual_bwd(t[f"ao.{i}"], t[f"inv2.{i}"], ssg1, dx, dbr, dssg1, B, L)
            ops.gemm_tn(dbr, t[f"y.{i}"], self.G(p + "attn.out_proj.weight"), dbias=self.G(p + "attn.out_proj.bias"))
            ops.gemm_nt(dbr, self.W(p + "attn.out_proj", T=True), None, dy)
            self.attn_bwd_launch(i, dy, delta, dqkv)
            ops.gemm_tn(dqkv, t[f"h1.{i}"], self.G(p + "attn.qkv_proj.weight"), dbias=self.G(p + "attn.qkv_proj.bias"))
            self.plain_gemm(dqkv, self.W(p + "attn.qkv_proj", T=True), None, dtmp)
            ops.gemm_tn(dtmp, a, self.G(p + "proj_cl.weight"), dbias=self.G(p + "proj_cl.bias"))
            ops.gemm_nt(dtmp, self.W(p + "proj_cl", T=True), None, da, accumulate=(i != self.depth - 1))
            ops.rmsnorm_film_bwd(t[f"x_in.{i}"], t[f"inv1.{i}"], ssg1, dtmp, dx, dssg1, B, L)
            lp = self.buf("d.lin_pre_ssg", (B, 3 * D), f32)
            self._det_flush(dssg1, dssg2)
            ops.linear_small_bwd(cg, self.P(p + "ssg2.weight"), None, dssg2, lp, self.G(p + "ssg2.weight"),
                                 self.G(p + "ssg2.bias"), dcg, True, OD_ACT_NONE)
            ops.linear_small_bwd(cg, self.P(p + "ssg1.weight"), None, dssg1, lp, self.G(p + "ssg1.weight"),
                                 self.G(p + "ssg1.bias"), dcg, True, OD_ACT_NONE)
            self._det_flush_segment(f"layer{i}")
            if reducer is not None:
                reducer.segment_done(f"layer{i}")

        ops.proj_in_bwd(xt, dx, self.G("proj_in.weight"), self.G("proj_in.bias"))
        da_pre = self.buf("d.a_pre", (self.Ma, A))
        ops.silu_bwd(self.ws.t["a_pre"], da, da_pre)
        ops.gemm_tn(da_pre, self.ws.t["a_t"], self.G("proj_audio.0.weight"), dbias=self.G("proj_audio.0.bias"))
        self._det_flush(dcg)
        ops.linear_small_bwd(style, self.P("proj_style.0.weight"), self.ws.t["cg_pre"], dcg,
                             self.buf("d.lin_pre_style", (B, self.Cg), f32), self.G("proj_style.0.weight"),
                             self.G("proj_style.0.bias"), None, False, OD_ACT_SILU)
        self._det_flush_segment("head")
        if reducer is not None:
            reducer.segment_done("head")
        if self.fused_attn_bwd() and self._attn_ws is not None and not self._attn_ws.checked:
            self._attn_ws.checked = True
            self.check_attn_status()

    def attn_status_ptr(self) -> int:
        return self._attn_ws.err_ptr() if self._attn_ws is not None else 0

    def attn_status_view(self) -> torch.Tensor:
        return self._attn_ws.err_view()

    ATTN_STATUS = {1: "a launch left jobs unprocessed (an XCD ran none of its workgroups): gradients incomplete",
                   2: "a launch with another (B, H, L) than the workspace's earlier launches was refused",
                   3: "a chain wait ran out of time (the predecessor's write never came; OD_FB_CHAIN_TIMEOUT_MS): dq is NaN"}

    def check_attn_status(self):
        if self._attn_ws is None:
            return
        code = 0
        for ws in {id(w): w for w in [self._attn_ws, *self._attn_ws_cache.values()]}.values():
            code = code or ws.status()
        if code != 0:
            raise RuntimeError(f"od_flash_attn_bwd_fused status {code}: {self.ATTN_STATUS.get(code, '?')}; the optimizer steps since then "
                               "were skipped.  OD_ATTN_BWD_FUSED=0 selects the two-kernel backward.")
```

osu_dreamer_amd/ops.py:

```python
from __future__ import annotations

import os
from typing import Optional

import torch

from . import _lib
from ._lib import OD_ACT_NONE, OD_ACT_SILU, OD_BF16, OD_EPI_NONE, OD_EPI_SILU, OD_F32, OD_F32X3, OD_F32X3W


def dt_code(dtype: torch.dtype) -> int:
    if dtype == torch.float32:
        return OD_F32
    if dtype == torch.bfloat16:
        return OD_BF16
    if dtype == torch.float16:
        return _lib.OD_F16
    raise TypeError(f"unsupported compute dtype {dtype}")


class SplitWeight:

    def __init__(self, storage: torch.Tensor):
        self.t = storage


def mm_code(dtype: torch.dtype, x3: bool, w=None) -> int:
    if isinstance(w, SplitWeight):
        if not (x3 and dtype == torch.float32):
            raise ValueError("a pre-split weight can only feed the fp32-as-3-x-bf16 product")
        return OD_F32X3W
    return OD_F32X3 if (x3 and dtype == torch.float32) else dt_code(dtype)


def _w(W):
    return W.t if isinstance(W, SplitWeight) else W


def _stream(t: torch.Tensor) -> int:
    return torch.cuda.current_stream(t.device).cuda_stream if t.is_cuda else 0


def _p(t: Optional[torch.Tensor]) -> Optional[int]:
    return None if t is None else t.data_ptr()


def _ld(t: torch.Tensor) -> int:
    assert t.dim() == 2 and t.stride(1) == 1, "need a row-major 2-D view"
    return t.stride(0)


def _f32(*ts):
    for t in ts:
        assert t is None or (t.dtype == torch.float32 and t.is_contiguous()), "expected contiguous fp32"


def _i32(*ts):
    for t in ts:
        assert t.dtype == torch.int32 and t.is_contiguous(), "expected contiguous int32"


def gemm_nt(A, W, bias, C, epilogue=OD_EPI_NONE, accumulate=False, x3=False):
    code, W = mm_code(A.dtype, x3, W), _w(W)
    M, K = A.shape
    N = W.shape[0]
    assert W.shape[1] == K and tuple(C.shape) == (M, N)
    assert A.dtype == W.dtype == C.dtype
    _f32(bias)
    _lib.lib().od_gemm_nt(code, _p(A), _ld(A), _p(W), _ld(W), _p(bias), _p(C), _ld(C), M, N, K,
                          epilogue, int(accumulate), _stream(A))


def gemm_nt_qkrope(A, W, bias, C, wq, wk, table, L, H, hd, eps, x3=False, q_scale=1.0):
    code, W = mm_code(A.dtype, x3, W), _w(W)
    M, K = A.shape
    N = W.shape[0]
    assert W.shape[1] == K and tuple(C.shape) == (M, N) and A.dtype == W.dtype == C.dtype
    _f32(bias, wq, wk, table)
    _lib.lib().od_gemm_nt_qkrope(code, _p(A), _ld(A), _p(W), _ld(W), _p(bias), _p(C), _ld(C), M, N, K,
                                 _p(wq), _p(wk), _p(table), L, H, hd, eps, q_scale, _stream(A))


def gemm_nt_qkrope_split(A, W, bias, C, qk_out, wq, wk, table, L, H, hd, eps, x3=False, q_scale=1.0):
    code, W = mm_code(A.dtype, x3, W), _w(W)
    M, K = A.shape
    N = W.shape[0]
    assert W.shape[1] == K and tuple(C.shape) == (M, N) and tuple(qk_out.shape) == (M, 2 * H * hd)
    assert A.dtype == W.dtype == C.dtype
    assert qk_out.dtype == A.dtype or (qk_out.dtype == torch.float16 and A.dtype == torch.bfloat16)
    _f32(bias, wq, wk, table)
    qk_code = _lib.OD_F16 if qk_out.dtype == torch.float16 else (OD_F32 if A.dtype == torch.float32 else code)
    _lib.lib().od_gemm_nt_qkrope_split(code, _p(A), _ld(A), _p(W), _ld(W), _p(bias), _p(C), _ld(C), _p(qk_out),
                                       _ld(qk_out), qk_code, M, N, K, _p(wq), _p(wk), _p(table), L, H, hd, eps, q_scale, _stream(A))


def gemm_tn(G, A, dW, n_cols=None, k_cols=None, dbias=None, n_block=0, n_valid=0):
    M = G.shape[0]
    N = n_cols if n_cols is not None else G.shape[1]
    K = k_cols if k_cols is not None else A.shape[1]
    rows = N if not n_block else (N // n_block) * n_valid
    assert not n_block or N % n_block == 0
    assert dW.dtype == torch.float32 and dW.is_contiguous() and dW.numel() == rows * K
    _f32(dbias)
    _lib.lib().od_gemm_tn_blocks(dt_code(G.dtype), _p(G), _ld(G), _p(A), _ld(A), _p(dW), K, _p(dbias), M, N, K, n_block, n_valid, _stream(G))


def colsum(G, out, n_cols=None):
    M = G.shape[0]
    N = n_cols if n_cols is not None else G.shape[1]
    _f32(out)
    _lib.lib().od_colsum(dt_code(G.dtype), _p(G), _ld(G), _p(out), M, N, _stream(G))


def pack_weight(src, dst, transpose=False, row_map=None):
    N = src.shape[0]
    K = src.numel() // N
    _f32(src)
    code = OD_F32X3W if isinstance(dst, SplitWeight) else dt_code(_w(dst).dtype)
    dst = _w(dst)
    if transpose:
        Kp, Np = dst.shape
    else:
        Np, Kp = dst.shape
    assert dst.is_contiguous()
    _lib.lib().od_pack_weight(code, _p(src), N, K, _p(dst), Np, Kp, int(transpose), _p(row_map), _stream(src))


def linear_small(x, W, b, out, pre=None, act=OD_ACT_NONE):
    B, K = x.shape
    N = W.shape[0]
    _f32(x, W, b, out, pre)
    _lib.lib().od_linear_small(_p(x), _p(W), _p(b), _p(out), _p(pre), B, N, K, act, _stream(x))


def linear_small_bwd(x, W, pre, dout, dpre, dW, db, dx, accumulate_dx, act=OD_ACT_NONE):
    B, K = x.shape
    N = W.shape[0]
    _f32(x, W, pre, dout, dpre, dW, db, dx)
    _lib.lib().od_linear_small_bwd(_p(x), _p(W), _p(pre), _p(dout), _p(dpre), _p(dW), _p(db), _p(dx),
                                   int(accumulate_dx), B, N, K, act, _stream(x))


def cl_to_frames(src, dst):
    B, C, L = src.shape
    _f32(src)
    _lib.lib().od_cl_to_frames(dt_code(dst.dtype), _p(src), _p(dst), _ld(dst), B, C, L, _stream(src))


def proj_in(xt, W, bias, x):
    B, E, L = xt.shape
    D = x.shape[1]
    _f32(xt, W, bias)
    _lib.lib().od_proj_in(dt_code(x.dtype), _p(xt), _p(W), _p(bias), _p(x), _ld(x), B, E, L, D, _stream(xt))


def proj_in_bwd(xt, dx, dW, db):
    B, E, L = xt.shape
    D = dx.shape[1]
    _f32(xt, dW, db)
    _lib.lib().od_proj_in_bwd(dt_code(dx.dtype), _p(xt), _p(dx), _ld(dx), _p(dW), _p(db), B, E, L, D, _stream(xt))


def silu(x, y):
    assert x.is_contiguous() and y.is_contiguous()
    _lib.lib().od_silu(dt_code(x.dtype), _p(x), _p(y), x.numel(), _stream(x))


def silu_bwd(x, dy, dx):
    assert x.is_contiguous() and dy.is_contiguous() and dx.is_contiguous()
    _lib.lib().od_silu_bwd(dt_code(x.dtype), _p(x), _p(dy), _p(dx), x.numel(), _stream(x))


def rmsnorm_film(x, ssg, cl, cl_bcast, h, inv_rms, B, L, eps=1e-6):
    C = x.shape[1]
    _f32(ssg, inv_rms)
    _lib.lib().od_rmsnorm_film(dt_code(x.dtype), _p(x), _ld(x), _p(ssg), _p(cl), _ld(cl) if cl is not None else 0,
                               int(cl_bcast), _p(h), _ld(h), _p(inv_rms), B, L, C, eps, _stream(x))


def rmsnorm_film_bwd(x, inv_rms, ssg, dh, dres, dssg, B, L):
    C = x.shape[1]
    _f32(ssg, inv_rms, dssg)
    _lib.lib().od_rmsnorm_film_bwd(dt_code(x.dtype), _p(x), _ld(x), _p(inv_rms), _p(ssg), _p(dh), _ld(dh), _p(dres),
                                   _ld(dres), _p(dssg), B, L, C, _stream(x))


def rmsnorm_gate_residual(x, h, ssg, xo, inv_rms, B, L, eps=1e-6):
    C = x.shape[1]
    _f32(ssg, inv_rms)
    _lib.lib().od_rmsnorm_gate_residual(dt_code(x.dtype), _p(x), _ld(x), _p(h), _ld(h), _p(ssg), _p(xo), _ld(xo),
                                        _p(inv_rms), B, L, C, eps, _stream(x))


def rmsnorm_gate_residual_film(x, h, ssg_a, xo, inv_a, ssg_b, cl, cl_bcast, h2, inv_b, B, L, eps=1e-6):
    _f32(ssg_a, ssg_b, inv_a, inv_b)
    _lib.lib().od_rmsnorm_gate_residual_film(dt_code(x.dtype), _p(x), _ld(x), _p(h), _ld(h), _p(ssg_a), _p(xo), _ld(xo),
                                             _p(inv_a), _p(ssg_b), _p(cl), _ld(cl) if cl is not None else 0, int(cl_bcast),
                                             _p(h2), _ld(h2), _p(inv_b), B, L, x.shape[1], eps, _stream(x))


def rmsnorm_gate_residual_film_dwconv(x, h, ssg_a, xo, inv_a, ssg_b, h2, inv_b, conv_w, conv_b, y, B, L, ksize, eps=1e-6):
    _f32(ssg_a, ssg_b, inv_a, inv_b, conv_w, conv_b)
    assert xo.data_ptr() != x.data_ptr() and xo.data_ptr() != h.data_ptr()
    _lib.lib().od_rmsnorm_gate_residual_film_dwconv(dt_code(x.dtype), _p(x), _ld(x), _p(h), _ld(h), _p(ssg_a), _p(xo), _ld(xo), _p(inv_a),
                                                    _p(ssg_b), _p(h2), _ld(h2) if h2 is not None else 0, _p(inv_b), _p(conv_w), _p(conv_b),
                                                    _p(y), _ld(y), B, L, x.shape[1], ksize, eps, _stream(x))


def rmsnorm_gate_residual_bwd(h, inv_rms, ssg, dy, dh, dssg, B, L):
    C = h.shape[1]
    _f32(ssg, inv_rms, dssg)
    _lib.lib().od_rmsnorm_gate_residual_bwd(dt_code(h.dtype), _p(h), _ld(h), _p(inv_rms), _p(ssg), _p(dy), _ld(dy),
                                            _p(dh), _ld(dh), _p(dssg), B, L, C, _stream(h))


def rope_table(table, L, hd):
    _f32(table)
    _lib.lib().od_rope_table(_p(table), L, hd, _stream(table))


def qk_norm_rope(qkv, wq, wk, table, qk_out, B, L, H, hd, eps, q_scale=1.0):
    _f32(wq, wk, table)
    _lib.lib().od_qk_norm_rope(dt_code(qkv.dtype), _p(qkv), _ld(qkv), _p(wq), _p(wk), _p(table), _p(qk_out),
                               _ld(qk_out), B, L, H, hd, eps, q_scale, _stream(qkv))


def qk_norm_rope_bwd(qkv, wq, wk, table, dqk, dqkv, dwq, dwk, B, L, H, hd, eps, q_scale=1.0):
    _f32(wq, wk, table, dwq, dwk)
    _lib.lib().od_qk_norm_rope_bwd(dt_code(qkv.dtype), _p(qkv), _ld(qkv), _p(wq), _p(wk), _p(table), _p(dqk), _ld(dqk),
                                   _p(dqkv), _ld(dqkv), _p(dwq), _p(dwk), B, L, H, hd, eps, q_scale, _stream(qkv))


def flash_attn_fwd(q, k, v, o, lse, B, H, L, hd, scale, x3=False, q_prescaled=False):
    _f32(lse)
    assert q.dtype == k.dtype == v.dtype and (o.dtype == q.dtype or (q.dtype == torch.float16 and o.dtype == torch.bfloat16))
    _lib.lib().od_flash_attn_fwd(mm_code(q.dtype, x3), _p(q), _ld(q), _p(k), _ld(k), _p(v), _ld(v), _p(o), _ld(o), _p(lse),
                                 B, H, L, hd, scale, int(q_prescaled), _stream(q))


class AttnAux:

    def __init__(self):
        import ctypes
        self.handle = ctypes.c_void_p()
        _lib.lib().od_attn_aux_create(ctypes.byref(self.handle))

    def close(self):
        if self.handle:
            _lib.lib().od_attn_aux_destroy(self.handle)
            self.handle = None

    def __del__(self):
        try:
            self.close()
        except Exception:
            pass


def flash_attn_fwd_varlen(q, k, v, o, lse, lens, B, H, L, hd, scale, x3=False, q_prescaled=False):
    _f32(lse)
    _i32(lens)
    assert q.dtype == k.dtype == v.dtype and (o.dtype == q.dtype or (q.dtype == torch.float16 and o.dtype == torch.bfloat16))
    _lib.lib().od_flash_attn_fwd_varlen(mm_code(q.dtype, x3), _p(q), _ld(q), _p(k), _ld(k), _p(v), _ld(v), _p(o), _ld(o), _p(lse),
                                        _p(lens), B, H, L, hd, scale, int(q_prescaled), _stream(q))


def flash_attn_bwd(q, k, v, o, do, lse, delta, dq, dk, dv, B, H, L, hd, scale, q_prescaled=False, aux=None):
    _f32(lse, delta)
    _lib.lib().od_flash_attn_bwd_aux(dt_code(q.dtype), _p(q), _ld(q), _p(k), _ld(k), _p(v), _ld(v), _p(o), _ld(o), _p(do),
                                     _ld(do), _p(lse), _p(delta), _p(dq), _ld(dq), _p(dk), _ld(dk), _p(dv), _ld(dv),
                                     B, H, L, hd, scale, int(q_prescaled), aux.handle if aux is not None else None, _stream(q))


class FusedAttnBwdWorkspace:

    def __init__(self, B, H, L, device, dtype=torch.bfloat16):
        import ctypes
        total, zero = ctypes.c_long(), ctypes.c_long()
        _lib.lib().od_flash_attn_bwd_fused_ws_bytes(dt_code(dtype), B, H, L, ctypes.byref(total), ctypes.byref(zero))
        self.shape = (B, H, L)
        self.dtype = dtype
        self.bytes = total.value
        assert zero.value <= self.bytes
        self.zero_bytes = zero.value
        self.buf = torch.empty(self.bytes, dtype=torch.uint8, device=device)
        self.reset()

    def reset(self):
        self.buf[:self.zero_bytes].zero_()

    def err_ptr(self) -> int:
        return self.buf.data_ptr() + int(_lib.lib().cdll.od_flash_attn_bwd_fused_err_offset())

    def err_view(self) -> torch.Tensor:
        off = int(_lib.lib().cdll.od_flash_attn_bwd_fused_err_offset())
        return self.buf[off:off + 4].view(torch.int32)

    def status(self) -> int:
        import ctypes
        err = ctypes.c_int(-1)
        _lib.lib().od_flash_attn_bwd_fused_status(_p(self.buf), ctypes.byref(err), _stream(self.buf))
        return err.value


def flash_attn_bwd_fused(q, k, v, o, do, lse, dq, dk, dv, B, H, L, hd, scale, ws: FusedAttnBwdWorkspace, q_prescaled=False):
    _f32(lse)
    assert ws.shape == (B, H, L), (ws.shape, (B, H, L))
    assert q.dtype == k.dtype == v.dtype and o.dtype == do.dtype == dq.dtype == dk.dtype == dv.dtype == torch.bfloat16
    assert q.dtype == torch.bfloat16 or (q.dtype == torch.float16 and ws.dtype == torch.float16)
    _lib.lib().od_flash_attn_bwd_fused(dt_code(q.dtype), _p(q), _ld(q), _p(k), _ld(k), _p(v), _ld(v), _p(o), _ld(o), _p(do), _ld(do),
                                       _p(lse), _p(dq), _ld(dq), _p(dk), _ld(dk), _p(dv), _ld(dv), B, H, L, hd, scale, int(q_prescaled),
                                       _p(ws.buf), ws.bytes, _stream(q))


def dwconv(x, w, bias, y, B, L, ksize):
    C = x.shape[1]
    _f32(w, bias)
    _lib.lib().od_dwconv(dt_code(x.dtype), _p(x), _ld(x), _p(w), _p(bias), _p(y), _ld(y), B, L, C, ksize, _stream(x))


def dwconv_varlen(x, w, bias, y, lens, B, L, ksize):
    C = x.shape[1]
    _f32(w, bias)
    _i32(lens)
    _lib.lib().od_dwconv_varlen(dt_code(x.dtype), _p(x), _ld(x), _p(w), _p(bias), _p(y), _ld(y), _p(lens), B, L, C, ksize, _stream(x))


def dwconv_bwd(x, w, dy, dx, dw, db, B, L, ksize):
    C = x.shape[1]
    _f32(w, dw, db)
    _lib.lib().od_dwconv_bwd(dt_code(x.dtype), _p(x), _ld(x), _p(w), _p(dy), _ld(dy), _p(dx), _ld(dx), _p(dw), _p(db),
                             B, L, C, ksize, _stream(x))


def scale_channels(x, scale, B, L):
    _f32(scale)
    assert scale.shape == (B, x.shape[1]) and scale.is_contiguous()
    _lib.lib().od_scale_channels(dt_code(x.dtype), _p(x), _ld(x), _p(scale), B, L, x.shape[1], _stream(x))


def swiglu_rmsnorm(vg, hh, inv_rms, Hf, Hp, eps=1e-6):
    _f32(inv_rms)
    _lib.lib().od_swiglu_rmsnorm(dt_code(vg.dtype), _p(vg), _ld(vg), _p(hh), _ld(hh), _p(inv_rms), vg.shape[0], Hf, Hp,
                                 eps, _stream(vg))


def swiglu_rmsnorm_bwd(vg, inv_rms, dhh, dvg, Hf, Hp):
    _f32(inv_rms)
    _lib.lib().od_swiglu_rmsnorm_bwd(dt_code(vg.dtype), _p(vg), _ld(vg), _p(inv_rms), _p(dhh), _ld(dhh), _p(dvg),
                                     _ld(dvg), vg.shape[0], Hf, Hp, _stream(vg))


def final_norm_proj_out(x, W, bias, v, inv_rms, B, L, eps=1e-6):
    C = x.shape[1]
    E = W.shape[0]
    _f32(W, bias, v, inv_rms)
    _lib.lib().od_final_norm_proj_out(dt_code(x.dtype), _p(x), _ld(x), _p(W), _p(bias), _p(v), _p(inv_rms), B, L, C, E,
                                      eps, _stream(x))


def final_norm_proj_out_bwd(x, inv_rms, W, dv, dx, dW, db, B, L):
    C = x.shape[1]
    E = W.shape[0]
    _f32(W, dv, inv_rms, dW, db)
    _lib.lib().od_final_norm_proj_out_bwd(dt_code(x.dtype), _p(x), _ld(x), _p(inv_rms), _p(W), _p(dv), _p(dx), _ld(dx),
                                          _p(dW), _p(db), B, L, C, E, _stream(x))


def uhead_fwd(xt, w, fsum, U):
    B, E, L = xt.shape
    _f32(xt, fsum, *w)
    _lib.lib().od_uhead_fwd(_p(xt), *[_p(t) for t in w], _p(fsum), B, E, L, U, _stream(xt))


def uhead_fwd_varlen(xt, w, fsum, lens, U):
    B, E, L = xt.shape
    _f32(xt, fsum, *w)
    _i32(lens)
    _lib.lib().od_uhead_fwd_varlen(_p(xt), *[_p(t) for t in w], _p(fsum), _p(lens), B, E, L, U, _stream(xt))


def uhead_bwd(xt, w, dfm, g, U):
    B, E, L = xt.shape
    _f32(xt, dfm, *w, *g)
    _lib.lib().od_uhead_bwd(_p(xt), *[_p(t) for t in w], _p(dfm), *[_p(t) for t in g], B, E, L, U, _stream(xt))


def uhead_tail(fsum, mod, w_out, b_out, u, L, u_scale):
    B, U = fsum.shape
    _f32(fsum, mod, w_out, b_out, u)
    _lib.lib().od_uhead_tail(_p(fsum), _p(mod), _p(w_out), _p(b_out), _p(u), B, U, L, u_scale, _stream(fsum))


def uhead_tail_varlen(fsum, mod, w_out, b_out, u, lens, L, u_scale):
    B, U = fsum.shape
    _f32(fsum, mod, w_out, b_out, u)
    _i32(lens)
    _lib.lib().od_uhead_tail_varlen(_p(fsum), _p(mod), _p(w_out), _p(b_out), _p(u), _p(lens), B, U, L, u_scale, _stream(fsum))


def uhead_tail_bwd(fsum, mod, w_out, b_out, du, dfm, dmod, dw_out, db_out, L, u_scale):
    B, U = fsum.shape
    _f32(fsum, mod, w_out, b_out, du, dfm, dmod, dw_out, db_out)
    _lib.lib().od_uhead_tail_bwd(_p(fsum), _p(mod), _p(w_out), _p(b_out), _p(du), _p(dfm), _p(dmod), _p(dw_out),
                                 _p(db_out), B, U, L, u_scale, _stream(fsum))


def make_xt(x0, x1, t, xt, dsq):
    B, E, L = x0.shape
    _f32(x0, x1, t, xt, dsq)
    _lib.lib().od_make_xt(_p(x0), _p(x1), _p(t), _p(xt), _p(dsq), B, E, L, _stream(x0))


def loss_grad(xt, x1, u, v, dsq, dv, sums, c0, osl_w, del_w):
    B, E, L = xt.shape
    _f32(xt, x1, u, v, dsq, dv, sums)
    _lib.lib().od_loss_grad(_p(xt), _p(x1), _p(u), _p(v), _p(dsq), _p(dv), _p(sums), B, E, L, c0, osl_w, del_w, _stream(xt))


def loss_finalize(sums, dsq, u, out, du, c0, osl_w, del_w):
    B = u.shape[0]
    _f32(sums, dsq, u, out, du)
    _lib.lib().od_loss_finalize(_p(sums), _p(dsq), _p(u), _p(out), _p(du), B, c0, osl_w, del_w, _stream(u))


def sampler_step(x, u, v, eta):
    B, E, L = x.shape
    _f32(x, u, v, eta)
    _lib.lib().od_sampler_step(_p(x), _p(u), _p(v), _p(eta), B, E, L, _stream(x))


def sampler_eta(u, eta, c0, num_steps):
    _f32(u, eta)
    _lib.lib().od_sampler_eta(_p(u), _p(eta), u.shape[0], c0, num_steps, _stream(u))


def sampler_eta_groups(u, offs, eta, c0, num_steps):
    _f32(u, eta)
    _i32(offs)
    G = offs.shape[0] - 1
    assert eta.numel() >= 2 * G
    _lib.lib().od_sampler_eta_groups(_p(u), _p(offs), _p(eta), G, c0, num_steps, _stream(u))


def sampler_step_varlen(x, u, v, eta, lens, offs):
    B, E, L = x.shape
    _f32(x, u, v, eta)
    _i32(lens, offs)
    _lib.lib().od_sampler_step_varlen(_p(x), _p(u), _p(v), _p(eta), _p(lens), _p(offs), offs.shape[0] - 1, B, E, L, _stream(x))


def sqnorm(g, out, status_ptr: int = 0):
    _f32(g, out)
    _lib.lib().od_sqnorm(_p(g), g.numel(), _p(out), status_ptr or None, _stream(g))


def adamw_ema(p, g, m, v, ema, lr, beta1, beta2, eps, weight_decay, step, ema_decay, ema_mode, gnorm_sq, max_norm, status_ptr: int = 0):
    _f32(p, g, m, v, ema, gnorm_sq)
    _lib.lib().od_adamw_ema(_p(p), _p(g), _p(m), _p(v), _p(ema), p.numel(), lr, beta1, beta2, eps, weight_decay, step,
                            ema_decay, ema_mode, _p(gnorm_sq), max_norm, status_ptr or None, _stream(p))


def ema_update(ema, p, decay, mode):
    _f32(ema, p)
    _lib.lib().od_ema_update(_p(ema), _p(p), p.numel(), decay, mode, _stream(p))


def style_conditioning(labels, rff_w, rff_b, cond_w, cond_b, null_labels, c):
    B, NL = labels.shape
    F, H = cond_w.shape[1], cond_w.shape[2]
    _f32(labels, rff_w, rff_b, cond_w, cond_b, null_labels, c)
    _lib.lib().od_style_conditioning(_p(labels), _p(rff_w), _p(rff_b), _p(cond_w), _p(cond_b), _p(null_labels), _p(c),
                                     B, NL, F, H, _stream(labels))


def rmsnorm_rows(x, gamma, y, eps):
    M, C = x.shape
    _f32(x, gamma, y)
    _lib.lib().od_rmsnorm_rows(_p(x), _p(gamma), _p(y), M, C, eps, _stream(x))


def style_conditioning_bwd(labels, rff_w, rff_b, dc, dcond_w, dcond_b, dnull_labels):
    B, NL = labels.shape
    F, H = dcond_w.shape[1], dcond_w.shape[2]
    _f32(labels, rff_w, rff_b, dc, dcond_w, dcond_b, dnull_labels)
    assert tuple(dc.shape) == (B, H) and rff_w.numel() == F and rff_b.numel() == F
    assert tuple(dcond_w.shape) == (NL, F, H) and tuple(dcond_b.shape) == (NL, H) and tuple(dnull_labels.shape) == (NL, H)
    _lib.lib().od_style_conditioning_bwd(_p(labels), _p(rff_w), _p(rff_b), _p(dc), _p(dcond_w), _p(dcond_b), _p(dnull_labels),
                                         B, NL, F, H, _stream(labels))


def rmsnorm_rows_bwd(x, gamma, dy, dx, dgamma, eps, accumulate_dx=False):
    M, C = x.shape
    _f32(x, gamma, dy, dx, dgamma)
    assert dy.shape == x.shape == dx.shape and (gamma is None or gamma.numel() == C) and (dgamma is None or dgamma.numel() == C)
    _lib.lib().od_rmsnorm_rows_bwd(_p(x), _p(gamma), _p(dy), _p(dx), _p(dgamma), M, C, eps, int(accumulate_dx), _stream(x))


def cast_rows(src, dst):
    assert src.is_contiguous() and dst.is_contiguous() and src.numel() == dst.numel()
    _lib.lib().od_cast_rows(dt_code(src.dtype), _p(src), dt_code(dst.dtype), _p(dst), src.numel(), _stream(src))


def spec_features_conv(audio, w1, b1, g1, w2, b2, g2, out, eps=1e-6):
    B, F, L = audio.shape
    _f32(audio, w1, b1, g1, w2, b2, g2)
    _lib.lib().od_spec_features_conv(dt_code(out.dtype), _p(audio), _p(w1), _p(b1), _p(g1), _p(w2), _p(b2), _p(g2),
                                     _p(out), _ld(out), B, F, L, eps, _stream(audio))


def rmsnorm_affine_film(x, gamma, ssg, y, B, L, act=OD_ACT_NONE, eps=1e-6):
    _f32(gamma, ssg)
    _lib.lib().od_rmsnorm_affine_film(dt_code(x.dtype), _p(x), _ld(x), _p(gamma), _p(ssg), _p(y), _ld(y), B, L, x.shape[1],
                                      eps, act, _stream(x))


def rmsnorm_affine_gate_residual(x, h, gamma, ssg, xo, B, L, eps=1e-6):
    _f32(gamma, ssg)
    _lib.lib().od_rmsnorm_affine_gate_residual(dt_code(x.dtype), _p(x), _ld(x), _p(h), _ld(h), _p(gamma), _p(ssg), _p(xo),
                                               _ld(xo), B, L, x.shape[1], eps, _stream(x))


def unet_mixer(x, p, p_bcast, gx, gamma, xo, B, L, eps=1e-6):
    _f32(gamma)
    _lib.lib().od_unet_mixer(dt_code(x.dtype), _p(x), _ld(x), _p(p), _ld(p), int(p_bcast), _p(gx), _ld(gx), _p(gamma),
                             _p(xo), _ld(xo), B, L, x.shape[1], eps, _stream(x))


def unet_down(x, w, bias, y, B, Lo, stride):
    _f32(w, bias)
    _lib.lib().od_unet_down(dt_code(x.dtype), _p(x), _ld(x), _p(w), _p(bias), _p(y), _ld(y), B, Lo, x.shape[1], stride,
                            _stream(x))


def unet_up(x, w, bias, y, B, Li, stride):
    _f32(w, bias)
    _lib.lib().od_unet_up(dt_code(x.dtype), _p(x), _ld(x), _p(w), _p(bias), _p(y), _ld(y), B, Li, x.shape[1], stride,
                          _stream(x))


def chart_head(x, W, bias, out, B, L, n_sigmoid, rms=False, eps=1e-6):
    _f32(W, bias, out)
    N = W.shape[0]
    _lib.lib().od_chart_head(dt_code(x.dtype), _p(x), _ld(x), _p(W), _p(bias), _p(out), B, L, x.shape[1], N, n_sigmoid,
                             int(rms), eps, _stream(x))


def attn_pool(scores, values, out, B, L, heads, hd):
    _f32(out)
    _lib.lib().od_attn_pool(dt_code(scores.dtype), _p(scores), _ld(scores), _p(values), _ld(values), _p(out), B, L, heads, hd,
                            _stream(scores))


def latent_bwd_ws_floats(kind, B, L, C, n=0):
    if kind == "spec":
        return B * -(-L // 32) * 4880
    f = _lib.lib().cdll.od_latent_bwd_block_frames(C)
    assert f > 0, "C must be a power of two in 8..512"
    per_row, flat = -(-L // f), -(-(B * L) // f)
    if kind == "film":
        return B * per_row * 3 * C
    if kind == "gate":
        return B * per_row * 2 * C
    if kind == "mixer":
        return (per_row if n else B * per_row) * C
    if kind in ("down", "up"):
        return flat * (2 * (n // 2) + 2) * C
    if kind == "head":
        return flat * n * (C + 1)
    raise ValueError(kind)


def rmsnorm_affine_film_bwd(x, gamma, ssg, dy, dx, dgamma, dssg, ws, B, L, act=OD_ACT_NONE, accumulate_dx=False, eps=1e-6):
    _f32(gamma, ssg, dgamma, dssg, ws)
    assert x.dtype == dy.dtype == dx.dtype
    _lib.lib().od_rmsnorm_affine_film_bwd(dt_code(x.dtype), _p(x), _ld(x), _p(gamma), _p(ssg), _p(dy), _ld(dy), _p(dx), _ld(dx),
                                          int(accumulate_dx), _p(dgamma), _p(dssg), _p(ws), ws.numel(), B, L, x.shape[1], eps, act,
                                          _stream(x))


def rmsnorm_affine_gate_residual_bwd(h, gamma, ssg, dxo, dh, dgamma, dssg, ws, B, L, eps=1e-6):
    _f32(gamma, ssg, dgamma, dssg, ws)
    assert h.dtype == dxo.dtype == dh.dtype
    _lib.lib().od_rmsnorm_affine_gate_residual_bwd(dt_code(h.dtype), _p(h), _ld(h), _p(gamma), _p(ssg), _p(dxo), _ld(dxo), _p(dh),
                                                   _ld(dh), _p(dgamma), _p(dssg), _p(ws), ws.numel(), B, L, h.shape[1], eps, _stream(h))


def unet_mixer_bwd(p, p_bcast, gx, gamma, dxo, dp, dgx, dgamma, ws, B, L, eps=1e-6):
    _f32(gamma, dgamma, ws)
    assert p.dtype == gx.dtype == dxo.dtype == dgx.dtype and dp.dtype == (torch.float32 if p_bcast else p.dtype)
    _lib.lib().od_unet_mixer_bwd(dt_code(p.dtype), _p(p), _ld(p), int(p_bcast), _p(gx), _ld(gx), _p(gamma), _p(dxo), _ld(dxo), _p(dp),
                                 _ld(dp), _p(dgx), _ld(dgx), _p(dgamma), _p(ws), ws.numel(), B, L, p.shape[1], eps, _stream(p))


def unet_down_bwd(x, w, dy, dx, dw, db, ws, B, Lo, stride):
    _f32(w, dw, db, ws)
    assert x.dtype == dy.dtype == dx.dtype
    _lib.lib().od_unet_down_bwd(dt_code(x.dtype), _p(x), _ld(x), _p(w), _p(dy), _ld(dy), _p(dx), _ld(dx), _p(dw), _p(db), _p(ws),
                                ws.numel(), B, Lo, x.shape[1], stride, _stream(x))


def unet_up_bwd(x, w, dy, dx, dw, db, ws, B, Li, stride):
    _f32(w, dw, db, ws)
    assert x.dtype == dy.dtype == dx.dtype
    _lib.lib().od_unet_up_bwd(dt_code(x.dtype), _p(x), _ld(x), _p(w), _p(dy), _ld(dy), _p(dx), _ld(dx), _p(dw), _p(db), _p(ws),
                              ws.numel(), B, Li, x.shape[1], stride, _stream(x))


def chart_head_bwd(x, W, bias, dout, dx, dW, db, ws, B, L, rms=False, eps=1e-6):
    _f32(W, bias, dout, dW, db, ws)
    N = W.shape[0]
    assert tuple(dout.shape) == (B, N, L) and x.dtype == dx.dtype
    _lib.lib().od_chart_head_bwd(dt_code(x.dtype), _p(x), _ld(x), _p(W), _p(bias), _p(dout), _p(dx), _ld(dx), _p(dW), _p(db), _p(ws),
                                 ws.numel(), B, L, x.shape[1], N, int(rms), eps, _stream(x))


def attn_pool_bwd(scores, values, dout, dscores, dvalues, B, L, heads, hd):
    _f32(dout)
    assert scores.dtype == values.dtype == dscores.dtype == dvalues.dtype
    _lib.lib().od_attn_pool_bwd(dt_code(scores.dtype), _p(scores), _ld(scores), _p(values), _ld(values), _p(dout), _p(dscores),
                                _ld(dscores), _p(dvalues), _ld(dvalues), B, L, heads, hd, _stream(scores))


def spec_features_conv_bwd(audio, w1, b1, g1, w2, b2, g2, dout, dw1, db1, dg1, dw2, db2, dg2, ws, eps=1e-6):
    B, F, L = audio.shape
    _f32(audio, w1, b1, g1, w2, b2, g2, dw1, db1, dg1, dw2, db2, dg2, ws)
    _lib.lib().od_spec_features_conv_bwd(dt_code(dout.dtype), _p(audio), _p(w1), _p(b1), _p(g1), _p(w2), _p(b2), _p(g2), _p(dout),
                                         _ld(dout), _p(dw1), _p(db1), _p(dg1), _p(dw2), _p(db2), _p(dg2), _p(ws), ws.numel(), B, F, L,
                                         eps, _stream(audio))


def add_rows(x, y):
    assert x.dtype == y.dtype and x.shape == y.shape and x.is_contiguous() and y.is_contiguous()
    _lib.lib().od_add_rows(dt_code(x.dtype), _p(x), _p(y), x.numel(), _stream(x))


def proj_in_bwd_input(dx, W, dxt):
    B, E, L = dxt.shape
    _f32(W, dxt)
    _lib.lib().od_proj_in_bwd_input(dt_code(dx.dtype), _p(dx), _ld(dx), _p(W), _p(dxt), B, E, L, dx.shape[1], _stream(dx))


def _lens(lens, B):
    _i32(lens)
    assert lens.dim() == 1 and lens.shape[0] == B and lens.is_contiguous(), "lens must be a contiguous int32 [B]"


def spec_features_conv_varlen(audio, w1, b1, g1, w2, b2, g2, out, lens, eps=1e-6):
    B, F, L = audio.shape
    _f32(audio, w1, b1, g1, w2, b2, g2)
    _lens(lens, B)
    _lib.lib().od_spec_features_conv_varlen(dt_code(out.dtype), _p(audio), _p(w1), _p(b1), _p(g1), _p(w2), _p(b2), _p(g2),
                                            _p(out), _ld(out), _p(lens), B, F, L, eps, _stream(audio))


def rmsnorm_affine_film_varlen(x, gamma, ssg, y, lens, B, L, act=OD_ACT_NONE, eps=1e-6):
    _f32(gamma, ssg)
    _lens(lens, B)
    _lib.lib().od_rmsnorm_affine_film_varlen(dt_code(x.dtype), _p(x), _ld(x), _p(gamma), _p(ssg), _p(y), _ld(y), _p(lens), B, L,
                                             x.shape[1], eps, act, _stream(x))


def unet_mixer_varlen(x, p, prow, gx, gamma, xo, B, L, eps=1e-6):
    _f32(gamma)
    _lens(prow, B)
    _lib.lib().od_unet_mixer_varlen(dt_code(x.dtype), _p(x), _ld(x), _p(p), _ld(p), _p(prow), _p(gx), _ld(gx), _p(gamma),
                                    _p(xo), _ld(xo), B, L, x.shape[1], eps, _stream(x))


def unet_down_varlen(x, w, bias, y, lens, B, Lo, stride):
    _f32(w, bias)
    _lens(lens, B)
    _lib.lib().od_unet_down_varlen(dt_code(x.dtype), _p(x), _ld(x), _p(w), _p(bias), _p(y), _ld(y), _p(lens), B, Lo, x.shape[1],
                                   stride, _stream(x))


def unet_up_varlen(x, w, bias, y, lens, B, Li, stride):
    _f32(w, bias)
    _lens(lens, B)
    _lib.lib().od_unet_up_varlen(dt_code(x.dtype), _p(x), _ld(x), _p(w), _p(bias), _p(y), _ld(y), _p(lens), B, Li, x.shape[1],
                                 stride, _stream(x))


def chart_head_varlen(x, W, bias, out, lens, B, L, n_sigmoid, rms=False, eps=1e-6):
    _f32(W, bias, out)
    _lens(lens, B)
    _lib.lib().od_chart_head_varlen(dt_code(x.dtype), _p(x), _ld(x), _p(W), _p(bias), _p(out), _p(lens), B, L, x.shape[1],
                                    W.shape[0], n_sigmoid, int(rms), eps, _stream(x))


def attn_pool_varlen(scores, values, out, lens, B, L, heads, hd):
    _f32(out)
    _lens(lens, B)
    _lib.lib().od_attn_pool_varlen(dt_code(scores.dtype), _p(scores), _ld(scores), _p(values), _ld(values), _p(out), _p(lens), B, L,
                                   heads, hd, _stream(scores))


def _u8(*ts):
    for t in ts:
        assert t.dtype == torch.uint8 and t.is_contiguous(), "expected contiguous uint8"


def mmd_imq(z, prior, out, dz, ws):
    N, D = z.shape
    _f32(z, prior, out, dz, ws)
    assert prior.shape == z.shape == dz.shape and out.numel() >= 4
    _lib.lib().od_mmd_imq(_p(z), _p(prior), _p(out), _p(dz), _p(ws), ws.numel(), N, D, _stream(z))


def scale_by(x, g, y):
    _f32(x, g, y)
    assert x.shape == y.shape
    _lib.lib().od_scale_by(_p(x), _p(g), _p(y), x.numel(), _stream(x))


def latent_perturb(z, s, eps_z, eps_s, u_s, repl, u_span, u_start, z_out, s_out, masked, start_span, s_noise, z_noise, s_mask_frac,
                   z_mask_frac, training):
    B2, E, l = z.shape
    S = s.shape[1]
    assert z.dtype == torch.float32
    _f32(s, eps_z, eps_s, u_s, repl, u_span, u_start, z_out, s_out)
    _u8(masked)
    _i32(start_span)
    assert tuple(z_out.shape) == (B2, E, l) and tuple(s_out.shape) == (B2, S) and masked.numel() == B2 and start_span.numel() == 2 * B2
    _lib.lib().od_latent_perturb(_p(z), z.stride(0), z.stride(1), z.stride(2), _p(s), _p(eps_z), _p(eps_s), _p(u_s), _p(repl), _p(u_span),
                                 _p(u_start), _p(z_out), _p(s_out), _p(masked), _p(start_span), B2, E, l, S, s_noise, z_noise,
                                 s_mask_frac, z_mask_frac, int(training), _stream(s))


def latent_perturb_bwd(dz_out, ds_out, masked, start_span, dz, ds):
    B2, E, l = dz_out.shape
    _f32(dz_out, ds_out, dz, ds)
    _u8(masked)
    _i32(start_span)
    _lib.lib().od_latent_perturb_bwd(_p(dz_out), _p(ds_out), _p(masked), _p(start_span), _p(dz), _p(ds), B2, E, l, ds_out.shape[1],
                                     _stream(ds))


def latent_loss_block_frames() -> int:
    return _lib.lib().cdll.od_latent_loss_block_frames()


def latent_loss_ws_floats(B2, L) -> int:
    return _lib.lib().cdll.od_latent_loss_ws_floats(B2, L)


def latent_loss(logits, chart, pred_labels, true_labels, masked, s_reg, loss_ema, ema_init, out, coef, ws, s_reg_weight, training):
    B2, C, L = logits.shape
    _f32(logits, chart, pred_labels, true_labels, s_reg, loss_ema, out, coef, ws)
    _u8(masked, ema_init)
    assert C == 9 and chart.shape == logits.shape and tuple(pred_labels.shape) == tuple(true_labels.shape) == (B2, 5)
    assert masked.numel() == B2 and loss_ema.numel() == 11 and out.numel() >= 13 and coef.numel() >= 11
    _lib.lib().od_latent_loss(_p(logits), _p(chart), _p(pred_labels), _p(true_labels), _p(masked), _p(s_reg), _p(loss_ema), _p(ema_init),
                              _p(out), _p(coef), _p(ws), ws.numel(), B2, L, s_reg_weight, int(training), _stream(logits))


def latent_loss_bwd(logits, chart, pred_labels, true_labels, masked, coef, g, dlogits, dlabels, ds_reg, s_reg_weight):
    B2, _, L = logits.shape
    _f32(logits, chart, pred_labels, true_labels, coef, g, dlogits, dlabels, ds_reg)
    _u8(masked)
    assert dlogits.shape == logits.shape and tuple(dlabels.shape) == (B2, 5)
    _lib.lib().od_latent_loss_bwd(_p(logits), _p(chart), _p(pred_labels), _p(true_labels), _p(masked), _p(coef), _p(g), _p(dlogits),
                                  _p(dlabels), _p(ds_reg), B2, L, s_reg_weight, _stream(logits))
```

Measured before the change: 3.022.

## Fuse FFN backward kernels: dwconv with rmsnorm-film bwd, bias folding, rowdot reuse

Result: no change. 3.022 (+0.0%).

```diff
diff --git a/include/osu_dreamer_hip.h b/include/osu_dreamer_hip.h
--- a/include/osu_dreamer_hip.h
+++ b/include/osu_dreamer_hip.h
@@ -55,12 +55,20 @@
 int od_rmsnorm_gate_residual_film(int dtype, const void* x, int ldx, const void* h, int ldh, const float* ssg_a, void* xo, int ldxo,
                                   float* inv_a, const float* ssg_b, const void* cl, int ldcl, int cl_bcast, void* h2, int ldh2,
                                   float* inv_b, int B, int L, int C, float eps, void* stream);
+int od_rmsnorm_gate_residual_hbias(int dtype, const void* x, int ldx, const void* h, int ldh, const float* hbias, const float* ssg, void* xo,
+                                   int ldxo, float* inv_rms, int B, int L, int C, float eps, void* stream);
+int od_rmsnorm_gate_residual_film_hbias(int dtype, const void* x, int ldx, const void* h, int ldh, const float* hbias, const float* ssg_a,
+                                        void* xo, int ldxo, float* inv_a, const float* ssg_b, const void* cl, int ldcl, int cl_bcast,
+                                        void* h2, int ldh2, float* inv_b, int B, int L, int C, float eps, void* stream);
 int od_rmsnorm_gate_residual_film_dwconv(int dtype, const void* x, int ldx, const void* h, int ldh, const float* ssg_a, void* xo, int ldxo,
                                          float* inv_a, const float* ssg_b, void* h2, int ldh2, float* inv_b, const float* conv_w,
                                          const float* conv_b, void* y, int ldy, int B, int L, int C, int ksize, float eps, void* stream);
 int od_rmsnorm_gate_residual_bwd(int dtype, const void* h, int ldh, const float* inv_rms, const float* ssg,
                                  const void* dy, int lddy, void* dh, int lddh, float* dssg, int B, int L, int C,
                                  void* stream);
+int od_rmsnorm_gate_residual_bwd_dot(int dtype, const void* h, int ldh, const float* inv_rms, const float* ssg,
+                                     const void* dy, int lddy, void* dh, int lddh, float* dssg, const float* bias,
+                                     float* rowdot, int B, int L, int C, void* stream);
 
 int od_rope_table(float* table, int L, int hd, void* stream);
 int od_qk_norm_rope(int dtype, const void* qkv, int ldqkv, const float* wq, const float* wk, const float* table,
@@ -96,11 +104,16 @@
                      int B, int L, int C, int ksize, void* stream);
 int od_dwconv_bwd(int dtype, const void* x, int ldx, const float* w, const void* dy, int lddy, void* dx, int lddx,
                   float* dw, float* db, int B, int L, int C, int ksize, void* stream);
+int od_dwconv_rmsnorm_film_bwd(int dtype, const void* h2, int ldh2, const float* conv_w, const void* dy, int lddy, const void* x, int ldx,
+                               const float* inv_rms, const float* ssg, void* dres, int lddres, float* dssg, float* dw, float* db,
+                               int B, int L, int C, int ksize, void* stream);
 int od_scale_channels(int dtype, void* x, int ldx, const float* scale, int B, int L, int C, void* stream);
 int od_swiglu_rmsnorm(int dtype, const void* vg, int ldvg, void* hh, int ldhh, float* inv_rms, int M, int Hf, int Hp,
                       float eps, void* stream);
 int od_swiglu_rmsnorm_bwd(int dtype, const void* vg, int ldvg, const float* inv_rms, const void* dhh, int lddhh,
                           void* dvg, int lddvg, int M, int Hf, int Hp, void* stream);
+int od_swiglu_rmsnorm_bwd_dot(int dtype, const void* vg, int ldvg, const float* inv_rms, const float* rowdot, const void* dhh,
+                              int lddhh, const float* mask, void* dvg, int lddvg, int B, int L, int Hf, int Hp, void* stream);
 
 int od_final_norm_proj_out(int dtype, const void* x, int ldx, const float* W, const float* bias, float* v,
                            float* inv_rms, int B, int L, int C, int E, float eps, void* stream);
diff --git a/osu_dreamer_amd/csrc/rowops.hip b/osu_dreamer_amd/csrc/rowops.hip
--- a/osu_dreamer_amd/csrc/rowops.hip
+++ b/osu_dreamer_amd/csrc/rowops.hip
@@ -18,6 +18,17 @@
 #pragma unroll
             for (int e = 0; e < 8; e++) v[i][e] = 0.f;
         }
+    }
+}
+template <int NCH>
+__device__ __forceinline__ void add_row_bias(const float* bias, int C, int lane, float (&v)[NCH][8]) {
+#pragma unroll
+    for (int i = 0; i < NCH; i++) {
+        const int c = (lane + 64 * i) * 8;
+        if (c >= C) continue;
+        float b[8]; od_ld8(bias + c, b);
+#pragma unroll
+        for (int e = 0; e < 8; e++) v[i][e] += b[e];
     }
 }
 template <int NCH>
@@ -130,16 +141,163 @@
     }
 }
 
-template <class T, int NCH>
+constexpr int FCB_RUN = 64;
+template <class T> struct raw_row;
+template <> struct raw_row<bf16_t> { u32x4 r; };
+template <> struct raw_row<float> { f32x4 r[2]; };
+__device__ __forceinline__ void raw_zero(raw_row<bf16_t>& a) { a.r = (u32x4)(0u); }
+__device__ __forceinline__ void raw_zero(raw_row<float>& a) { a.r[0] = (f32x4)(0.f); a.r[1] = (f32x4)(0.f); }
+__device__ __forceinline__ void raw_load(raw_row<bf16_t>& a, const bf16_t* p) { a.r = *(const u32x4*)p; }
+__device__ __forceinline__ void raw_load(raw_row<float>& a, const float* p) { a.r[0] = *(const f32x4*)p; a.r[1] = *(const f32x4*)(p + 4); }
+__device__ __forceinline__ void raw_unpack(const raw_row<bf16_t>& a, float (&v)[8]) {
+#pragma unroll
+    for (int i = 0; i < 4; i++) {
+        union { uint32_t u; float f; } lo, hi;
+        lo.u = a.r[i] << 16; hi.u = a.r[i] & 0xffff0000u;
+        v[2 * i] = lo.f; v[2 * i + 1] = hi.f;
+    }
+}
+__device__ __forceinline__ void raw_unpack(const raw_row<float>& a, float (&v)[8]) {
+#pragma unroll
+    for (int i = 0; i < 4; i++) { v[i] = a.r[0][i]; v[4 + i] = a.r[1][i]; }
+}
+
+template <class T, int KS>
+__global__ __launch_bounds__(256) void dwconv_rmsnorm_film_bwd_kernel(const T* __restrict__ h2, int ldh2, const float* __restrict__ w,
+                                                                      const T* __restrict__ dy, int lddy, const T* __restrict__ x, int ldx,
+                                                                      const float* __restrict__ inv_rms, const float* __restrict__ ssg,
+                                                                      T* __restrict__ dres, int lddres, float* __restrict__ dssg,
+                                                                      float* __restrict__ dw, float* __restrict__ db, int L, int C,
+                                                                      const OdDetTable* __restrict__ det) {
+    constexpr int R = KS / 2;
+    __shared__ long long redw[512 * (KS + 1)];
+    __shared__ float red[2][512];
+    __shared__ int s_bad;
+    const int lane = threadIdx.x & 63, wave = threadIdx.x >> 6;
+    const int b = blockIdx.y;
+    const int l0 = (blockIdx.x * 4 + wave) * FCB_RUN;
+    const int lend = l0 + FCB_RUN < L ? l0 + FCB_RUN : L;
+    const int c = lane * 8;
+    const bool act = c < C;
+    for (int i = threadIdx.x; i < C * (KS + 1); i += 256) redw[i] = 0;
+    if (threadIdx.x == 0) s_bad = 0;
+    __syncthreads();
+    float wv[8][KS], adw[8][KS], adb[8], scl[8], dsc[8], dsh[8];
+#pragma unroll
+    for (int k = 0; k < 8; k++) {
+        adb[k] = 0.f; scl[k] = 0.f; dsc[k] = 0.f; dsh[k] = 0.f;
+#pragma unroll
+        for (int j = 0; j < KS; j++) { wv[k][j] = act ? w[(size_t)(c + k) * KS + j] : 0.f; adw[k][j] = 0.f; }
+    }
+    if (act) od_ld8(ssg + (size_t)b * 3 * C + c, scl);
+    if (l0 < L) {
+        const T* yb = dy + (size_t)b * L * lddy + c;
+        float wy[KS][8];
+#pragma unroll
+        for (int j = 0; j < KS - 1; j++) {
+            const int l = l0 - R + j;
+            if (act && l >= 0 && l < L) od_ld8(yb + (size_t)l * lddy, wy[j]);
+            else {
+#pragma unroll
+                for (int k = 0; k < 8; k++) wy[j][k] = 0.f;
+            }
+        }
+        raw_row<T> py, ph, px, pd;
+        float pinv;
+        raw_zero(py); raw_zero(ph); raw_zero(px); raw_zero(pd);
+        auto fetch = [&](int l) {
+            const size_t m = (size_t)b * L + l;
+            pinv = inv_rms[m];
+            if (act) {
+                raw_load(ph, h2 + m * ldh2 + c);
+                raw_load(px, x + m * ldx + c);
+                raw_load(pd, dres + m * lddres + c);
+                if (l + R < L) raw_load(py, yb + (size_t)(l + R) * lddy); else raw_zero(py);
+            }
+        };
+        fetch(l0);
+        for (int l = l0; l < lend; l++) {
+            const size_t m = (size_t)b * L + l;
+            float hv[8], xv[8], o[8], gv[8];
+            raw_unpack(py, wy[KS - 1]);
+            raw_unpack(ph, hv);
+            raw_unpack(px, xv);
+            raw_unpack(pd, o);
+            const float inv = pinv;
+            if (l + 1 < lend) fetch(l + 1);
+            float dot = 0.f;
+#pragma unroll
+            for (int k = 0; k < 8; k++) {
+                float sacc = 0.f;
+#pragma unroll
+                for (int jj = 0; jj < KS; jj++) sacc += wv[k][jj] * wy[KS - 1 - jj][k];
+                gv[k] = od_round_to<T>(sacc);
+                adb[k] += wy[R][k];
+#pragma unroll
+                for (int jj = 0; jj < KS; jj++) adw[k][jj] += wy[KS - 1 - jj][k] * hv[k];
+            }
+#pragma unroll
+            for (int e = 0; e < 8; e++) {
+                const float xh = xv[e] * inv;
+                dsc[e] += gv[e] * xh;
+                dsh[e] += gv[e];
+                gv[e] *= (1.f + scl[e]);
+                dot += gv[e] * xh;
+                xv[e] = xh;
+            }
+            dot = od_wave_sum(dot) / (float)C;
+#pragma unroll
+            for (int e = 0; e < 8; e++) o[e] += inv * (gv[e] - xv[e] * dot);
+            if (act) od_st8(dres + m * lddres + c, o);
+#pragma unroll
+            for (int j = 0; j < KS - 1; j++)
+#pragma unroll
+                for (int k = 0; k < 8; k++) wy[j][k] = wy[j + 1][k];
+        }
+        if (act) {
+#pragma unroll
+            for (int k = 0; k < 8; k++) {
+                od_lds_fix_add(&redw[(c + k) * (KS + 1) + KS], adb[k], &s_bad);
+#pragma unroll
+                for (int j = 0; j < KS; j++) od_lds_fix_add(&redw[(c + k) * (KS + 1) + j], adw[k][j], &s_bad);
+            }
+        }
+    }
+    for (int wi = 0; wi < 4; wi++) {
+        if (wave == wi) {
+#pragma unroll
+            for (int e = 0; e < 8; e++) {
+                if (wi == 0) { red[0][c + e] = dsc[e]; red[1][c + e] = dsh[e]; }
+                else { red[0][c + e] += dsc[e]; red[1][c + e] += dsh[e]; }
+            }
+        }
+        __syncthreads();
+    }
+    for (int i = threadIdx.x; i < C; i += 256) {
+        od_red_add(det, dssg + (size_t)b * 3 * C + i, red[0][i]);
+        od_red_add(det, dssg + (size_t)b * 3 * C + C + i, red[1][i]);
+    }
+    for (int i = threadIdx.x; i < C * (KS + 1); i += 256) {
+        const int ch = i / (KS + 1), j = i % (KS + 1);
+        const float v = od_lds_unfix(redw[i], s_bad);
+        if (v != 0.f) {
+            if (j == KS) od_red_add(det, db + ch, v); else od_red_add(det, dw + (size_t)ch * KS + j, v);
+        }
+    }
+}
+
+template <class T, int NCH, bool HB = false>
 __global__ __launch_bounds__(256) void rmsnorm_gate_res_kernel(const T* __restrict__ x, int ldx, const T* __restrict__ h, int ldh,
                                                                const float* __restrict__ ssg, T* __restrict__ xo, int ldxo,
-                                                               float* __restrict__ inv_rms, int B, int L, int C, float eps) {
+                                                               float* __restrict__ inv_rms, int B, int L, int C, float eps,
+                                                               const float* __restrict__ hbias = nullptr) {
     const int lane = threadIdx.x & 63;
     const long m = (long)blockIdx.x * 4 + (threadIdx.x >> 6);
     if (m >= (long)B * L) return;
     const int b = (int)(m / L);
     float v[NCH][8];
     load_row<T, NCH>(h + m * ldh, C, lane, v);
+    if constexpr (HB) add_row_bias<NCH>(hbias, C, lane, v);
     const float inv = rsqrtf(row_sumsq<NCH>(v) / (float)C + eps);
     if (lane == 0 && inv_rms) inv_rms[m] = inv;
     const float* gate = ssg + (size_t)b * 3 * C + 2 * C;
@@ -156,19 +314,20 @@
     }
 }
 
-template <class T, int NCH>
+template <class T, int NCH, bool HB = false>
 __global__ __launch_bounds__(256) void rmsnorm_gate_res_film_kernel(const T* __restrict__ x, int ldx, const T* __restrict__ h, int ldh,
                                                                     const float* __restrict__ ssg_a, T* __restrict__ xo, int ldxo,
                                                                     float* __restrict__ inv_a, const float* __restrict__ ssg_b,
                                                                     const T* __restrict__ cl, int ldcl, int cl_bcast,
                                                                     T* __restrict__ h2, int ldh2, float* __restrict__ inv_b,
-                                                                    int B, int L, int C, float eps) {
+                                                                    int B, int L, int C, float eps, const float* __restrict__ hbias = nullptr) {
     const int lane = threadIdx.x & 63;
     const long m = (long)blockIdx.x * 4 + (threadIdx.x >> 6);
     if (m >= (long)B * L) return;
     const int b = (int)(m / L), l = (int)(m % L);
     float v[NCH][8];
     load_row<T, NCH>(h + m * ldh, C, lane, v);
+    if constexpr (HB) add_row_bias<NCH>(hbias, C, lane, v);
     const float inv = rsqrtf(row_sumsq<NCH>(v) / (float)C + eps);
     if (lane == 0 && inv_a) inv_a[m] = inv;
     const float* gate = ssg_a + (size_t)b * 3 * C + 2 * C;
@@ -298,28 +457,41 @@
     }
 }
 
-template <class T, int NCH>
+#if defined(OD_EMU)
+#define RGB_FMA(a, b, c) ((a) * (b) + (c))
+#else
+#define RGB_FMA(a, b, c) __builtin_fmaf((a), (b), (c))
+#endif
+template <class T, int NCH, bool ROWDOT = false>
 __global__ __launch_bounds__(256) void rmsnorm_gate_res_bwd_kernel(const T* __restrict__ h, int ldh, const float* __restrict__ inv_rms,
                                                                    const float* __restrict__ ssg, const T* __restrict__ dy, int lddy,
                                                                    T* __restrict__ dh, int lddh, float* __restrict__ dssg,
-                                                                   int B, int L, int C, const OdDetTable* __restrict__ det) {
+                                                                   int B, int L, int C, const OdDetTable* __restrict__ det,
+                                                                   const float* __restrict__ bias = nullptr,
+                                                                   float* __restrict__ rowdot = nullptr) {
     __shared__ float red[NCH * 512];
     const int lane = threadIdx.x & 63, wave = threadIdx.x >> 6;
     const int b = blockIdx.y;
     const int l0 = (blockIdx.x * 4 + wave) * ROWS_PER_WAVE_BWD;
     float dg[NCH][8], gate[NCH][8];
+    float bv[NCH][8];
+    const bool hb = ROWDOT && bias != nullptr;
 #pragma unroll
     for (int i = 0; i < NCH; i++) {
         const int c = (lane + 64 * i) * 8;
 #pragma unroll
         for (int e = 0; e < 8; e++) { dg[i][e] = 0.f; gate[i][e] = 0.f; }
         if (c < C) od_ld8(ssg + (size_t)b * 3 * C + 2 * C + c, gate[i]);
+#pragma unroll
+        for (int e = 0; e < 8; e++) bv[i][e] = 0.f;
+        if (hb && c < C) od_ld8(bias + c, bv[i]);
     }
     for (int r = 0; r < ROWS_PER_WAVE_BWD; r++) {
         const int l = l0 + r;
         if (l >= L) break;
         const long m = (long)b * L + l;
         float hv[NCH][8], gv[NCH][8];
+        float hr[ROWDOT ? NCH : 1][8];
         load_row<T, NCH>(h + m * ldh, C, lane, hv);
         load_row<T, NCH>(dy + m * lddy, C, lane, gv);
         const float inv = inv_rms[m];
@@ -328,21 +500,44 @@
         for (int i = 0; i < NCH; i++)
 #pragma unroll
             for (int e = 0; e < 8; e++) {
+                if constexpr (ROWDOT) {
+                    hr[i][e] = hv[i][e];
+                    if (hb) hv[i][e] += bv[i][e];
+                }
                 const float hh = hv[i][e] * inv;
-                dg[i][e] += gv[i][e] * hh;
-                gv[i][e] *= gate[i][e];
-                dot += gv[i][e] * hh;
+                if constexpr (ROWDOT) {
+#pragma clang fp contract(off)
+                    dg[i][e] = RGB_FMA(gv[i][e], hh, dg[i][e]);
+                    gv[i][e] *= gate[i][e];
+                    dot += gv[i][e] * hh;
+                } else {
+                    dg[i][e] += gv[i][e] * hh;
+                    gv[i][e] *= gate[i][e];
+                    dot += gv[i][e] * hh;
+                }
                 hv[i][e] = hh;
             }
         dot = od_wave_sum(dot) / (float)C;
+        float rd = 0.f;
 #pragma unroll
         for (int i = 0; i < NCH; i++) {
             const int c = (lane + 64 * i) * 8;
             if (c >= C) continue;
             float o[8];
 #pragma unroll
-            for (int e = 0; e < 8; e++) o[e] = inv * (gv[i][e] - hv[i][e] * dot);
+            for (int e = 0; e < 8; e++) {
+                if constexpr (ROWDOT) o[e] = inv * RGB_FMA(-hv[i][e], dot, gv[i][e]);
+                else o[e] = inv * (gv[i][e] - hv[i][e] * dot);
+            }
             od_st8(dh + m * lddh + c, o);
+            if constexpr (ROWDOT) {
+#pragma unroll
+                for (int e = 0; e < 8; e++) rd += od_round_to<T>(o[e]) * hr[i][e];
+            }
+        }
+        if constexpr (ROWDOT) {
+            rd = od_wave_sum(rd);
+            if (lane == 0) rowdot[m] = rd;
         }
     }
     for (int w = 0; w < 4; w++) {
@@ -424,6 +619,44 @@
         od_st8(dvg + m * lddvg + c, ov);
         od_st8(dvg + m * lddvg + Hp + c, og);
     }
+}
+
+template <class T>
+__global__ __launch_bounds__(256) void swiglu_rmsnorm_bwd_dot_kernel(const T* __restrict__ vg, int ldvg, const float* __restrict__ inv_rms,
+                                                                     const float* __restrict__ rowdot, const T* __restrict__ dhh, int lddhh,
+                                                                     const float* __restrict__ mask, T* __restrict__ dvg, int lddvg,
+                                                                     long M, int L, int Hf, int Hp) {
+    const int cpr = Hp >> 3;
+    const long first = (long)blockIdx.x * 256;
+    const long m0 = first / cpr;
+    const int r = (int)(first - m0 * cpr) + (int)threadIdx.x;
+    const long m = m0 + r / cpr;
+    if (m >= M) return;
+    const int c = (r % cpr) * 8;
+    float v[8], g[8], d[8];
+    od_ld8(vg + m * ldvg + c, v);
+    od_ld8(vg + m * ldvg + Hp + c, g);
+    od_ld8(dhh + m * lddhh + c, d);
+    if (mask) {
+        float mk[8];
+        od_ld8(mask + (m / L) * Hp + c, mk);
+#pragma unroll
+        for (int e = 0; e < 8; e++) d[e] *= mk[e];
+    }
+    const float inv = inv_rms[m];
+    const float dot = rowdot[m] / (float)Hf;
+    float ov[8], og[8];
+#pragma unroll
+    for (int e = 0; e < 8; e++) {
+        const float gs = od_sigmoid(g[e]);
+        const float sg = g[e] * gs;
+        const float sh = v[e] * sg * inv;
+        const float ds = inv * (d[e] - sh * dot);
+        ov[e] = ds * sg;
+        og[e] = ds * v[e] * (gs * (1.0f + g[e] * (1.0f - gs)));
+    }
+    od_st8(dvg + m * lddvg + c, ov);
+    od_st8(dvg + m * lddvg + Hp + c, og);
 }
 
 template <class T, int NCH>
@@ -862,6 +1095,23 @@
     return 0;
 }
 
+extern "C" int od_dwconv_rmsnorm_film_bwd(int dtype, const void* h2, int ldh2, const float* conv_w, const void* dy, int lddy, const void* x,
+                                          int ldx, const float* inv_rms, const float* ssg, void* dres, int lddres, float* dssg,
+                                          float* dw, float* db, int B, int L, int C, int ksize, void* stream) {
+    if (C % 8 || ldh2 % 8 || lddy % 8 || ldx % 8 || lddres % 8) return OD_ERR_ALIGN;
+    if (C > 512 || (ksize != 3 && ksize != 5 && ksize != 7 && ksize != 9)) return OD_ERR_UNSUPPORTED;
+    if (!h2 || !conv_w || !dy || !x || !inv_rms || !ssg || !dres || !dssg || !dw || !db || dres == dy) return OD_ERR_ARG;
+    dim3 grid((unsigned)((L + 4 * FCB_RUN - 1) / (4 * FCB_RUN)), (unsigned)B);
+#define FCB_GO1(T_, KS_) OD_LAUNCH((dwconv_rmsnorm_film_bwd_kernel<T_, KS_>), grid, dim3(256), 0, (hipStream_t)stream, (const T_*)h2, ldh2, conv_w, \
+                   (const T_*)dy, lddy, (const T_*)x, ldx, inv_rms, ssg, (T_*)dres, lddres, dssg, dw, db, L, C, od_det_active())
+#define FCB_GO(KS_) do { if (dtype == OD_BF16) FCB_GO1(bf16_t, KS_); else if (dtype == OD_F32) FCB_GO1(float, KS_); else return OD_ERR_ARG; } while (0)
+    if (ksize == 5) FCB_GO(5); else if (ksize == 3) FCB_GO(3); else if (ksize == 7) FCB_GO(7); else FCB_GO(9);
+#undef FCB_GO
+#undef FCB_GO1
+    OD_CHECK_LAUNCH();
+    return 0;
+}
+
 extern "C" int od_rmsnorm_gate_residual(int dtype, const void* x, int ldx, const void* h, int ldh, const float* ssg, void* xo,
                                         int ldxo, float* inv_rms, int B, int L, int C, float eps, void* stream) {
     if (C % 8 || ldx % 8 || ldh % 8 || ldxo % 8) return OD_ERR_ALIGN;
@@ -883,6 +1133,34 @@
     DISPATCH_T_NCH(dtype, nch_for(C),
         OD_LAUNCH((rmsnorm_gate_res_film_kernel<T_, N_>), grid, dim3(256), 0, (hipStream_t)stream, (const T_*)x, ldx, (const T_*)h, ldh,
                   ssg_a, (T_*)xo, ldxo, inv_a, ssg_b, (const T_*)cl, ldcl, cl_bcast, (T_*)h2, ldh2, inv_b, B, L, C, eps));
+    OD_CHECK_LAUNCH();
+    return 0;
+}
+
+extern "C" int od_rmsnorm_gate_residual_hbias(int dtype, const void* x, int ldx, const void* h, int ldh, const float* hbias, const float* ssg,
+                                              void* xo, int ldxo, float* inv_rms, int B, int L, int C, float eps, void* stream) {
+    if (C % 8 || ldx % 8 || ldh % 8 || ldxo % 8) return OD_ERR_ALIGN;
+    if (!hbias) return OD_ERR_ARG;
+    const long M = (long)B * L;
+    dim3 grid((unsigned)((M + 3) / 4));
+    DISPATCH_T_NCH(dtype, nch_for(C),
+        OD_LAUNCH((rmsnorm_gate_res_kernel<T_, N_, true>), grid, dim3(256), 0, (hipStream_t)stream, (const T_*)x, ldx, (const T_*)h, ldh, ssg,
+                  (T_*)xo, ldxo, inv_rms, B, L, C, eps, hbias));
+    OD_CHECK_LAUNCH();
+    return 0;
+}
+
+extern "C" int od_rmsnorm_gate_residual_film_hbias(int dtype, const void* x, int ldx, const void* h, int ldh, const float* hbias,
+                                                   const float* ssg_a, void* xo, int ldxo, float* inv_a, const float* ssg_b, const void* cl,
+                                                   int ldcl, int cl_bcast, void* h2, int ldh2, float* inv_b, int B, int L, int C, float eps,
+                                                   void* stream) {
+    if (C % 8 || ldx % 8 || ldh % 8 || ldxo % 8 || ldh2 % 8 || (cl && ldcl % 8)) return OD_ERR_ALIGN;
+    if (!hbias) return OD_ERR_ARG;
+    const long M = (long)B * L;
+    dim3 grid((unsigned)((M + 3) / 4));
+    DISPATCH_T_NCH(dtype, nch_for(C),
+        OD_LAUNCH((rmsnorm_gate_res_film_kernel<T_, N_, true>), grid, dim3(256), 0, (hipStream_t)stream, (const T_*)x, ldx, (const T_*)h, ldh,
+                  ssg_a, (T_*)xo, ldxo, inv_a, ssg_b, (const T_*)cl, ldcl, cl_bcast, (T_*)h2, ldh2, inv_b, B, L, C, eps, hbias));
     OD_CHECK_LAUNCH();
     return 0;
 }
@@ -924,6 +1202,19 @@
     return 0;
 }
 
+extern "C" int od_rmsnorm_gate_residual_bwd_dot(int dtype, const void* h, int ldh, const float* inv_rms, const float* ssg,
+                                                const void* dy, int lddy, void* dh, int lddh, float* dssg, const float* bias,
+                                                float* rowdot, int B, int L, int C, void* stream) {
+    if (C % 8 || ldh % 8 || lddy % 8 || lddh % 8) return OD_ERR_ALIGN;
+    if (!rowdot) return OD_ERR_ARG;
+    dim3 grid((L + 4 * ROWS_PER_WAVE_BWD - 1) / (4 * ROWS_PER_WAVE_BWD), B);
+    DISPATCH_T_NCH(dtype, nch_for(C),
+        OD_LAUNCH((rmsnorm_gate_res_bwd_kernel<T_, N_, true>), grid, dim3(256), 0, (hipStream_t)stream, (const T_*)h, ldh, inv_rms, ssg,
+                  (const T_*)dy, lddy, (T_*)dh, lddh, dssg, B, L, C, od_det_active(), bias, rowdot));
+    OD_CHECK_LAUNCH();
+    return 0;
+}
+
 extern "C" int od_swiglu_rmsnorm(int dtype, const void* vg, int ldvg, void* hh, int ldhh, float* inv_rms, int M, int Hf, int Hp,
                                  float eps, void* stream) {
     if (Hp % 8 || ldvg % 8 || ldhh % 8 || Hf > Hp) return OD_ERR_ALIGN;
@@ -942,6 +1233,25 @@
     DISPATCH_T_NCH(dtype, nch_for(Hp),
         OD_LAUNCH((swiglu_rmsnorm_bwd_kernel<T_, N_>), grid, dim3(256), 0, (hipStream_t)stream, (const T_*)vg, ldvg, inv_rms,
                   (const T_*)dhh, lddhh, (T_*)dvg, lddvg, (long)M, Hf, Hp));
+    OD_CHECK_LAUNCH();
+    return 0;
+}
+
+extern "C" int od_swiglu_rmsnorm_bwd_dot(int dtype, const void* vg, int ldvg, const float* inv_rms, const float* rowdot, const void* dhh,
+                                         int lddhh, const float* mask, void* dvg, int lddvg, int B, int L, int Hf, int Hp, void* stream) {
+    if (Hp % 8 || ldvg % 8 || lddhh % 8 || lddvg % 8 || Hf > Hp) return OD_ERR_ALIGN;
+    if (!rowdot || B < 1 || L < 1 || Hp < 8) return OD_ERR_ARG;
+    const long M = (long)B * L;
+    const long chunks = M * (Hp / 8);
+    if ((chunks + 255) / 256 > 0x7fffffffL) return OD_ERR_UNSUPPORTED;
+    dim3 grid((unsigned)((chunks + 255) / 256));
+    if (dtype == OD_BF16)
+        OD_LAUNCH((swiglu_rmsnorm_bwd_dot_kernel<bf16_t>), grid, dim3(256), 0, (hipStream_t)stream, (const bf16_t*)vg, ldvg, inv_rms, rowdot,
+                  (const bf16_t*)dhh, lddhh, mask, (bf16_t*)dvg, lddvg, M, L, Hf, Hp);
+    else if (dtype == OD_F32)
+        OD_LAUNCH((swiglu_rmsnorm_bwd_dot_kernel<float>), grid, dim3(256), 0, (hipStream_t)stream, (const float*)vg, ldvg, inv_rms, rowdot,
+                  (const float*)dhh, lddhh, mask, (float*)dvg, lddvg, M, L, Hf, Hp);
+    else return OD_ERR_ARG;
     OD_CHECK_LAUNCH();
     return 0;
 }
diff --git a/osu_dreamer_amd/engine.py b/osu_dreamer_amd/engine.py
--- a/osu_dreamer_amd/engine.py
+++ b/osu_dreamer_amd/engine.py
@@ -273,15 +273,16 @@
             if self._drop_active():
                 ops.scale_channels(hh, self.draw_dropout_mask(i), B, L)
             fo = self.lbuf("fo", i, (M, D))
-            self.plain_gemm(hh, self.W(p + "ffn.proj_o"), self.P(p + "ffn.proj_o.bias"), fo)
+            fo_bias = self.P(p + "ffn.proj_o.bias") if self.train else None
+            self.plain_gemm(hh, self.W(p + "ffn.proj_o"), None if self.train else self.P(p + "ffn.proj_o.bias"), fo)
             x = self.buf(f"x_in.{i + 1}", (M, D)) if self.train else self.buf(f"x_in.{(i + 1) & 1}", (M, D))
             if i + 1 < self.depth:
                 h1 = self.lbuf("h1", i + 1, (M, D))
                 ops.rmsnorm_gate_residual_film(x_mid, fo, ssg2, x, self.lbuf("inv5", i, (M,), f32),
                                                self.ws.t[f"ssg1.{i + 1}"], cl_of(i + 1), bcast, h1,
-                                               self.lbuf("inv1", i + 1, (M,), f32), B, L)
-            else:
-                ops.rmsnorm_gate_residual(x_mid, fo, ssg2, x, self.lbuf("inv5", i, (M,), f32), B, L)
+                                               self.lbuf("inv1", i + 1, (M,), f32), B, L, h_bias=fo_bias)
+            else:
+                ops.rmsnorm_gate_residual(x_mid, fo, ssg2, x, self.lbuf("inv5", i, (M,), f32), B, L, h_bias=fo_bias)
         self._x_last = x
         ops.final_norm_proj_out(x, self.P("proj_out.weight"), self.P("proj_out.bias"), v,
                                 self.buf("invf", (M,), f32), B, L)
@@ -381,6 +382,7 @@
         dqkv = self.buf("d.qkv", (M, 3 * dh))
         da = self.buf("d.a", (self.Ma, A))
         delta = self.buf("d.delta", (B, self.H, L), f32)
+        rowdot = self.buf("d.rowdot", (M,), f32)
         dcg = self.buf("d.cg", (B, self.Cg), f32)
         dssg1, dssg2 = self.buf("d.ssg1", (B, 3 * D), f32), self.buf("d.ssg2", (B, 3 * D), f32)
 
@@ -402,23 +404,28 @@
             ssg1, ssg2 = t[f"ssg1.{i}"], t[f"ssg2.{i}"]
             dssg1.zero_()
             dssg2.zero_()
-            ops.rmsnorm_gate_residual_bwd(t[f"fo.{i}"], t[f"inv5.{i}"], ssg2, dx, dbr, dssg2, B, L)
+            ops.rmsnorm_gate_residual_bwd_dot(t[f"fo.{i}"], t[f"inv5.{i}"], ssg2, dx, dbr, dssg2, self.P(p + "ffn.proj_o.bias"), rowdot, B, L)
             ops.gemm_tn(dbr, t[f"hh.{i}"], self.G(p + "ffn.proj_o.weight"), n_cols=D, k_cols=Hf,
                         dbias=self.G(p + "ffn.proj_o.bias"))
             ops.gemm_nt(dbr, self.W(p + "ffn.proj_o", T=True), None, dhh)
-            if self._drop_active():
-                ops.scale_channels(dhh, self._drop_mask(i), B, L)
-            ops.swiglu_rmsnorm_bwd(t[f"vg.{i}"], t[f"inv4.{i}"], dhh, dvg, Hf, Hp)
+            ops.swiglu_rmsnorm_bwd_dot(t[f"vg.{i}"], t[f"inv4.{i}"], rowdot, dhh, self._drop_mask(i) if self._drop_active() else None,
+                                       dvg, Hf, Hp, B, L)
             gw, gb = self.G(p + "ffn.proj_vg.1.weight"), self.G(p + "ffn.proj_vg.1.bias")
             hdw = t[f"hdw.{i}"] if self.radius > 0 else t[f"h2.{i}"]
             ops.gemm_tn(dvg, hdw, gw, n_cols=2 * Hp, k_cols=D, dbias=gb, n_block=Hp, n_valid=Hf)
             if self.radius > 0:
                 self.plain_gemm(dvg, self.W(p + "ffn.proj_vg.1", T=True), None, dtmp)
-                ops.dwconv_bwd(t[f"h2.{i}"], self.P(p + "ffn.proj_vg.0.weight"), dtmp, dbr,
-                               self.G(p + "ffn.proj_vg.0.weight"), self.G(p + "ffn.proj_vg.0.bias"), B, L, self.ksize)
+                if D <= 512:
+                    ops.dwconv_rmsnorm_film_bwd(t[f"h2.{i}"], self.P(p + "ffn.proj_vg.0.weight"), dtmp, t[f"x_mid.{i}"], t[f"inv3.{i}"],
+                                                ssg2, dx, dssg2, self.G(p + "ffn.proj_vg.0.weight"), self.G(p + "ffn.proj_vg.0.bias"),
+                                                B, L, self.ksize)
+                else:
+                    ops.dwconv_bwd(t[f"h2.{i}"], self.P(p + "ffn.proj_vg.0.weight"), dtmp, dbr,
+                                   self.G(p + "ffn.proj_vg.0.weight"), self.G(p + "ffn.proj_vg.0.bias"), B, L, self.ksize)
+                    ops.rmsnorm_film_bwd(t[f"x_mid.{i}"], t[f"inv3.{i}"], ssg2, dbr, dx, dssg2, B, L)
             else:
                 self.plain_gemm(dvg, self.W(p + "ffn.proj_vg.1", T=True), None, dbr)
-            ops.rmsnorm_film_bwd(t[f"x_mid.{i}"], t[f"inv3.{i}"], ssg2, dbr, dx, dssg2, B, L)
+                ops.rmsnorm_film_bwd(t[f"x_mid.{i}"], t[f"inv3.{i}"], ssg2, dbr, dx, dssg2, B, L)
             ops.rmsnorm_gate_residual_bwd(t[f"ao.{i}"], t[f"inv2.{i}"], ssg1, dx, dbr, dssg1, B, L)
             ops.gemm_tn(dbr, t[f"y.{i}"], self.G(p + "attn.out_proj.weight"), dbias=self.G(p + "attn.out_proj.bias"))
             ops.gemm_nt(dbr, self.W(p + "attn.out_proj", T=True), None, dy)
diff --git a/osu_dreamer_amd/ops.py b/osu_dreamer_amd/ops.py
--- a/osu_dreamer_amd/ops.py
+++ b/osu_dreamer_amd/ops.py
@@ -185,15 +185,26 @@
                                    _ld(dres), _p(dssg), B, L, C, _stream(x))
 
 
-def rmsnorm_gate_residual(x, h, ssg, xo, inv_rms, B, L, eps=1e-6):
-    C = x.shape[1]
-    _f32(ssg, inv_rms)
+def rmsnorm_gate_residual(x, h, ssg, xo, inv_rms, B, L, eps=1e-6, h_bias=None):
+    C = x.shape[1]
+    _f32(ssg, inv_rms, h_bias)
+    if h_bias is not None:
+        assert h_bias.numel() == C
+        _lib.lib().od_rmsnorm_gate_residual_hbias(dt_code(x.dtype), _p(x), _ld(x), _p(h), _ld(h), _p(h_bias), _p(ssg), _p(xo), _ld(xo),
+                                                  _p(inv_rms), B, L, C, eps, _stream(x))
+        return
     _lib.lib().od_rmsnorm_gate_residual(dt_code(x.dtype), _p(x), _ld(x), _p(h), _ld(h), _p(ssg), _p(xo), _ld(xo),
                                         _p(inv_rms), B, L, C, eps, _stream(x))
 
 
-def rmsnorm_gate_residual_film(x, h, ssg_a, xo, inv_a, ssg_b, cl, cl_bcast, h2, inv_b, B, L, eps=1e-6):
-    _f32(ssg_a, ssg_b, inv_a, inv_b)
+def rmsnorm_gate_residual_film(x, h, ssg_a, xo, inv_a, ssg_b, cl, cl_bcast, h2, inv_b, B, L, eps=1e-6, h_bias=None):
+    _f32(ssg_a, ssg_b, inv_a, inv_b, h_bias)
+    if h_bias is not None:
+        assert h_bias.numel() == x.shape[1]
+        _lib.lib().od_rmsnorm_gate_residual_film_hbias(dt_code(x.dtype), _p(x), _ld(x), _p(h), _ld(h), _p(h_bias), _p(ssg_a), _p(xo), _ld(xo),
+                                                       _p(inv_a), _p(ssg_b), _p(cl), _ld(cl) if cl is not None else 0, int(cl_bcast),
+                                                       _p(h2), _ld(h2), _p(inv_b), B, L, x.shape[1], eps, _stream(x))
+        return
     _lib.lib().od_rmsnorm_gate_residual_film(dt_code(x.dtype), _p(x), _ld(x), _p(h), _ld(h), _p(ssg_a), _p(xo), _ld(xo),
                                              _p(inv_a), _p(ssg_b), _p(cl), _ld(cl) if cl is not None else 0, int(cl_bcast),
                                              _p(h2), _ld(h2), _p(inv_b), B, L, x.shape[1], eps, _stream(x))
@@ -212,6 +223,14 @@
     _f32(ssg, inv_rms, dssg)
     _lib.lib().od_rmsnorm_gate_residual_bwd(dt_code(h.dtype), _p(h), _ld(h), _p(inv_rms), _p(ssg), _p(dy), _ld(dy),
                                             _p(dh), _ld(dh), _p(dssg), B, L, C, _stream(h))
+
+
+def rmsnorm_gate_residual_bwd_dot(h, inv_rms, ssg, dy, dh, dssg, bias, rowdot, B, L):
+    C = h.shape[1]
+    _f32(ssg, inv_rms, dssg, rowdot, bias)
+    assert rowdot.numel() == B * L and rowdot.is_contiguous() and (bias is None or (bias.numel() == C and bias.is_contiguous()))
+    _lib.lib().od_rmsnorm_gate_residual_bwd_dot(dt_code(h.dtype), _p(h), _ld(h), _p(inv_rms), _p(ssg), _p(dy), _ld(dy),
+                                                _p(dh), _ld(dh), _p(dssg), _p(bias), _p(rowdot), B, L, C, _stream(h))
 
 
 def rope_table(table, L, hd):
@@ -333,6 +352,13 @@
                              B, L, C, ksize, _stream(x))
 
 
+def dwconv_rmsnorm_film_bwd(h2, w, dy, x, inv_rms, ssg, dres, dssg, dw, db, B, L, ksize):
+    C = x.shape[1]
+    _f32(w, inv_rms, ssg, dssg, dw, db)
+    _lib.lib().od_dwconv_rmsnorm_film_bwd(dt_code(x.dtype), _p(h2), _ld(h2), _p(w), _p(dy), _ld(dy), _p(x), _ld(x), _p(inv_rms), _p(ssg),
+                                          _p(dres), _ld(dres), _p(dssg), _p(dw), _p(db), B, L, C, ksize, _stream(x))
+
+
 def scale_channels(x, scale, B, L):
     _f32(scale)
     assert scale.shape == (B, x.shape[1]) and scale.is_contiguous()
@@ -349,6 +375,13 @@
     _f32(inv_rms)
     _lib.lib().od_swiglu_rmsnorm_bwd(dt_code(vg.dtype), _p(vg), _ld(vg), _p(inv_rms), _p(dhh), _ld(dhh), _p(dvg),
                                      _ld(dvg), vg.shape[0], Hf, Hp, _stream(vg))
+
+
+def swiglu_rmsnorm_bwd_dot(vg, inv_rms, rowdot, dhh, mask, dvg, Hf, Hp, B, L):
+    _f32(inv_rms, rowdot, mask)
+    assert vg.shape[0] == B * L and rowdot.numel() == B * L and (mask is None or (mask.shape == (B, Hp) and mask.is_contiguous()))
+    _lib.lib().od_swiglu_rmsnorm_bwd_dot(dt_code(vg.dtype), _p(vg), _ld(vg), _p(inv_rms), _p(rowdot), _p(dhh), _ld(dhh), _p(mask),
+                                         _p(dvg), _ld(dvg), B, L, Hf, Hp, _stream(vg))
 
 
 def final_norm_proj_out(x, W, bias, v, inv_rms, B, L, eps=1e-6):
```
